# cloudflare/zkp-ecdsa

Hardware: NVIDIA H100
Metric: ZKAttest proofs/sec (higher is better)
Workload: dtype u256/u258 (32-bit limbs, Montgomery)

## Files before the change

__graft_entry__.py:

```python
from __future__ import annotations

import hashlib
import os
import subprocess
import sys

ROOT = os.path.dirname(os.path.abspath(__file__))
CSRC = os.path.join(ROOT, 'zkp_ecdsa_b200', 'csrc')
LIB = os.path.join(ROOT, 'zkp_ecdsa_b200', 'libzkattest.so')
LIB_WAR = os.path.join(ROOT, 'zkp_ecdsa_b200', 'libzkattest_war256.so')
HOSTSIM = os.path.join(ROOT, 'tests', 'hostsim', 'libzkattest_hostsim.so')
HOSTSIM_WAR = os.path.join(ROOT, 'tests', 'hostsim', 'libzkattest_hostsim_war256.so')
PROBE_SRC = os.path.join(ROOT, 'tests', 'probe', 'zk_probe.cu')
PROBE = os.path.join(ROOT, 'tests', 'probe', 'libzkprobe.so')
PROBE_HOST = os.path.join(ROOT, 'tests', 'probe', 'libzkprobe_host.so')
PROBE_JAC_SRC = os.path.join(ROOT, 'tests', 'probe', 'zk_probe_jac.cu')
PROBE_JAC = os.path.join(ROOT, 'tests', 'probe', 'libzkprobe_jac.so')
PROBE_JAC_HOST = os.path.join(ROOT, 'tests', 'probe', 'libzkprobe_jac_host.so')
PROBE_SEED_SRC = os.path.join(ROOT, 'tests', 'probe', 'zk_probe_seed.cu')
PROBE_SEED = os.path.join(ROOT, 'tests', 'probe', 'libzkprobe_seed.so')
PROBE_SEED_HOST = os.path.join(ROOT, 'tests', 'probe', 'libzkprobe_seed_host.so')
PROBE_SHAPE_SRC = os.path.join(ROOT, 'tests', 'probe', 'zk_probe_shape.cu')
PROBE_SHAPE = os.path.join(ROOT, 'tests', 'probe', 'libzkprobe_shape.so')
PROBE_SHAPE_HOST = os.path.join(ROOT, 'tests', 'probe', 'libzkprobe_shape_host.so')
ORACLE_CPU = os.path.join(ROOT, 'oracle', '_ref', 'libzkattest_cpu.so')
ARCH = ['-gencode', 'arch=compute_90a,code=sm_90a']
NVCC_FLAGS = ARCH + ['-O3', '-std=c++17', '-lineinfo',
              '--compiler-options', '-fPIC', '-shared']


def _sources():
    return sorted(os.path.join(CSRC, f) for f in os.listdir(CSRC) if f.endswith(('.cu', '.cuh', '.h', '.inc')))


def _stamp(extra='', files=()):
    h = hashlib.sha256(extra.encode())
    for p in _sources() + [os.path.join(ROOT, 'include', 'zkattest.h')] + list(files):
        h.update(p.encode())
        h.update(open(p, 'rb').read())
    return h.hexdigest()


def _build_if_stale(out, cmd, tag, files=()):
    stamp_file = out + '.stamp'
    stamp = _stamp(' '.join(cmd), files)
    if os.path.exists(out) and os.path.exists(stamp_file) and open(stamp_file).read() == stamp:
        return False
    print(f'[build] {tag}: {" ".join(cmd)}', flush=True)
    tmp = out + '.tmp'
    subprocess.check_call([tmp if c == out else c for c in cmd], cwd=ROOT)
    os.replace(tmp, out)
    open(stamp_file, 'w').write(stamp)
    return True


def build_lib():
    nvcc = os.environ.get('NVCC', '/usr/local/cuda/bin/nvcc')
    cmd = [nvcc] + NVCC_FLAGS + ['-I' + os.path.join(ROOT, 'include'), '-I' + CSRC, '-o', LIB,
                                 os.path.join(CSRC, 'zkattest.cu')]
    return _build_if_stale(LIB, cmd, 'libzkattest.so (sm_90a)')


def build_lib_war():
    nvcc = os.environ.get('NVCC', '/usr/local/cuda/bin/nvcc')
    cmd = [nvcc] + NVCC_FLAGS + ['-DZKA_PG_WAR256', '-I' + os.path.join(ROOT, 'include'), '-I' + CSRC, '-o', LIB_WAR,
                                 os.path.join(CSRC, 'zkattest.cu')]
    return _build_if_stale(LIB_WAR, cmd, 'libzkattest_war256.so (sm_90a)')


def build_hostsim(war=False):
    out = HOSTSIM_WAR if war else HOSTSIM
    os.makedirs(os.path.dirname(out), exist_ok=True)
    cmd = ['g++', '-std=c++17', '-O2', '-DZKA_HOSTSIM'] + (['-DZKA_PG_WAR256'] if war else []) + [
        '-x', 'c++', '-I' + os.path.join(ROOT, 'include'), '-I' + CSRC, '-fPIC', '-shared', '-o', out,
        os.path.join(CSRC, 'zkattest.cu')]
    return _build_if_stale(out, cmd, 'hostsim war256 (tests only)' if war else 'hostsim (tests only)')


def build_probe(host=False, jac=False):
    out = (PROBE_JAC_HOST if host else PROBE_JAC) if jac else (PROBE_HOST if host else PROBE)
    src = PROBE_JAC_SRC if jac else PROBE_SRC
    if host:
        cmd = ['g++', '-std=c++17', '-O2', '-DZKA_HOSTSIM', '-x', 'c++', '-fPIC', '-shared']
    else:
        cmd = [os.environ.get('NVCC', '/usr/local/cuda/bin/nvcc')] + NVCC_FLAGS
    cmd += ['-I' + os.path.join(ROOT, 'include'), '-I' + CSRC, '-o', out, src]
    tag = ('probe_jac' if jac else 'probe') + (' host (tests only)' if host else ' (sm_90a, tests only)')
    return _build_if_stale(out, cmd, tag, [PROBE_SRC, PROBE_JAC_SRC] if jac else [PROBE_SRC])


def build_probe_seed(host=False):
    out = PROBE_SEED_HOST if host else PROBE_SEED
    if host:
        cmd = ['g++', '-std=c++17', '-O2', '-DZKA_HOSTSIM', '-x', 'c++', '-fPIC', '-shared']
    else:
        cmd = [os.environ.get('NVCC', '/usr/local/cuda/bin/nvcc')] + NVCC_FLAGS
    cmd += ['-I' + os.path.join(ROOT, 'include'), '-I' + CSRC, '-o', out, PROBE_SEED_SRC]
    return _build_if_stale(out, cmd, 'probe_seed' + (' host (tests only)' if host else ' (sm_90a, tests only)'), [PROBE_SEED_SRC])


def build_probe_shape(host=False):
    out = PROBE_SHAPE_HOST if host else PROBE_SHAPE
    if host:
        cmd = ['g++', '-std=c++17', '-O2', '-DZKA_HOSTSIM', '-x', 'c++', '-fPIC', '-shared']
    else:
        cmd = [os.environ.get('NVCC', '/usr/local/cuda/bin/nvcc')] + NVCC_FLAGS
    cmd += ['-I' + os.path.join(ROOT, 'include'), '-I' + CSRC, '-o', out, PROBE_SHAPE_SRC]
    return _build_if_stale(out, cmd, 'probe_shape' + (' host (tests only)' if host else ' (sm_90a, tests only)'), [PROBE_SHAPE_SRC])


def build_oracle_cpu():
    src = os.path.join(ROOT, 'oracle', 'cpu', 'zkattest_cpu.cpp')
    hdr = os.path.join(ROOT, 'include', 'zkattest.h')
    if os.path.exists(ORACLE_CPU) and os.path.getmtime(ORACLE_CPU) >= max(os.path.getmtime(src), os.path.getmtime(hdr)):
        return False
    print('[build] oracle/cpu -> oracle/_ref/libzkattest_cpu.so', flush=True)
    subprocess.check_call(['make', '-C', os.path.join(ROOT, 'oracle', 'cpu')])
    return True


def build_tools():
    nvcc = os.environ.get('NVCC', '/usr/local/cuda/bin/nvcc')
    tdir = os.path.join(ROOT, 'tools')
    for name in ('imad_peak', 'mul_peak'):
        src, out = os.path.join(tdir, name + '.cu'), os.path.join(tdir, name)
        if not os.path.exists(src):
            continue
        if os.path.exists(out) and os.path.getmtime(out) >= max(os.path.getmtime(p) for p in _sources() + [src]):
            continue
        cmd = [nvcc] + ARCH + ['-O3', '-std=c++17', '-I' + CSRC,
               '-I' + os.path.join(ROOT, 'include'), '-o', out, src]
        print(f'[build] tools/{name}: {" ".join(cmd)}', flush=True)
        subprocess.check_call(cmd, cwd=ROOT)


def build() -> None:
    from concurrent.futures import ThreadPoolExecutor
    jobs = [build_lib, build_lib_war, build_hostsim, lambda: build_hostsim(war=True), build_oracle_cpu, build_tools,
            build_probe, lambda: build_probe(host=True), lambda: build_probe(jac=True),
            lambda: build_probe(host=True, jac=True), build_probe_seed, lambda: build_probe_seed(host=True),
            build_probe_shape, lambda: build_probe_shape(host=True)]
    with ThreadPoolExecutor(max_workers=min(len(jobs), max(1, (os.cpu_count() or 2)))) as ex:
        for f in [ex.submit(j) for j in jobs]:
            f.result()
    sys.path.insert(0, ROOT)
    import zkp_ecdsa_b200
    import oracle


def smoke() -> None:
    sys.path.insert(0, ROOT)
    import numpy as np
    from zkp_ecdsa_b200 import api, synth
    from oracle import flat
    from oracle import zkattest as OZ
    from oracle.big import Tape

    eng = api.Engine(device=0)
    rnd = synth.params_rnd(1)
    params = eng.generate_params_list(rnd=rnd)
    wl = synth.Workload(B=2, N=8, seed=1)
    tape = synth.random_tape(2, eng.lib.prove_tape_len(8), seed=2)
    res = eng.prove_batch(params, wl.msg_hash, wl.sig, wl.pk, wl.which, wl.ring, tape)
    assert (res.status == 0).all(), res.status
    oparams = OZ.generate_params_list(Tape(rnd))
    for b in range(2):
        pr = OZ.prove_signature_list(oparams, wl.msg_hash[b].tobytes(), wl.sig[b].tobytes(), wl.pk[b].tobytes(),
                                     int(wl.which[b]), wl.ring_ints(), Tape(tape[b].tobytes()))
        assert flat.ser_proof(pr) == res.proof_bytes(b), f'proof {b} differs from the oracle'
    from oracle import seed_tape as ST
    seed = bytes(range(32))
    rs = eng.prove_batch_seeded(params, wl.msg_hash[:1], wl.sig[:1], wl.pk[:1], wl.which[:1], wl.ring,
                                np.frombuffer(seed, np.uint8).reshape(1, 32).copy())
    assert rs.status[0] == 0, rs.status
    pr = OZ.prove_signature_list(oparams, wl.msg_hash[0].tobytes(), wl.sig[0].tobytes(), wl.pk[0].tobytes(),
                                 int(wl.which[0]), wl.ring_ints(), Tape(ST.prove_tape(seed, 80, 3)))
    assert flat.ser_proof(pr) == rs.proof_bytes(0), 'seeded proof differs from the oracle on the expanded tape'
    from zkp_ecdsa_b200 import verify_tape as VT
    vts = eng.lib.verify_tape_len(8, 80)
    ok = np.zeros(2, np.uint8)
    st = np.zeros(2, np.int32)
    eng.lib.verify_batch(params.handle, 2, wl.msg_hash, wl.ring, 8, res.proofs, res.proofs.shape[1], res.proof_len,
                         VT.random_verify_tape(2, vts, 8, 80, seed=3), vts, ok, st)
    assert list(ok) == [1, 1] and not st.any(), (ok, st)
    rw = synth.RingsWorkload(2, [17, 5], [1, 0], seed=5)
    rings = eng.load_rings(rw.rings)
    rt = synth.random_tape(2, eng.lib.prove_tape_len(17), seed=6)
    rr = eng.prove_batch_rings(params, rings, rw.ring_of, rw.msg_hash, rw.sig, rw.pk, rw.which, rt)
    assert (rr.status == 0).all(), rr.status
    for b in range(2):
        pr = OZ.prove_signature_list(oparams, rw.msg_hash[b].tobytes(), rw.sig[b].tobytes(), rw.pk[b].tobytes(),
                                     int(rw.which[b]), rw.ring_ints(int(rw.ring_of[b])), Tape(rt[b].tobytes()))
        assert flat.ser_proof(pr) == rr.proof_bytes(b), f'ring-set proof {b} differs from the oracle'
    rings.close()
    launched = eng.lib.launch_count()
    war = ''
    if os.path.exists(LIB_WAR):
        from oracle.curves import tomEdwards256, war256
        ew = api.Engine(device=0, proof_group='war256')
        pw = ew.generate_params_list(16, rnd=rnd)
        tw = synth.random_tape(1, ew.lib.prove_tape_len(8, 16), seed=4)
        rw = ew.prove_batch(pw, wl.msg_hash[:1], wl.sig[:1], wl.pk[:1], wl.which[:1], wl.ring, tw)
        assert (rw.status == 0).all(), rw.status
        flat.set_proof_group(war256)
        try:
            ow = OZ.generate_params_list(Tape(rnd), 16, war256)
            pr = OZ.prove_signature_list(ow, wl.msg_hash[0].tobytes(), wl.sig[0].tobytes(), wl.pk[0].tobytes(),
                                         int(wl.which[0]), wl.ring_ints(), Tape(tw[0].tobytes()))
            assert flat.ser_proof(pr) == rw.proof_bytes(0), 'war256 proof differs from the oracle'
        finally:
            flat.set_proof_group(tomEdwards256)
        launched += ew.lib.launch_count()
        war = '; war256 build: 1 proof bit-exact'
    print(f'smoke ok: 2 proofs bit-exact vs oracle and accepted by the verifier, 1 seeded proof bit-exact, '
          f'2 ring-set proofs over rings of depths 3 and 5 bit-exact{war}; '
          'kernels launched:', launched)


if __name__ == '__main__':
    build()
    if len(sys.argv) > 1 and sys.argv[1] == 'smoke':
        smoke()
```

zkp_ecdsa_b200/capi.py:

```python
from __future__ import annotations

import ctypes as C
import os
from typing import Optional

import numpy as np

_HERE = os.path.dirname(os.path.abspath(__file__))
DEFAULT_LIB = os.path.join(_HERE, 'libzkattest.so')

SYMBOLS = [
    'zka_init', 'zka_shutdown', 'zka_last_error', 'zka_version', 'zka_launch_count',
    'zka_params_generate', 'zka_params_create', 'zka_params_destroy', 'zka_key_to_int',
    'zka_proof_max_len', 'zka_prove_tape_len', 'zka_verify_tape_len',
    'zka_prove_batch', 'zka_verify_batch',
    'zka_tom_commit_batch', 'zka_p256_mul_batch', 'zka_field_op_batch', 'zka_hash80_batch',
    'zka_get_stream', 'zka_set_profiling', 'zka_profile_reset', 'zka_profile_json', 'zka_config',
    'zka_lanes', 'zka_set_option', 'zka_proofs_pack', 'zka_proofs_unpack', 'zka_verify_batch_ex', 'zka_verify_tape_len_ex',
    'zka_verify_exp_batch', 'zka_verify_membership_batch', 'zka_verify_equality_batch', 'zka_verify_mult_batch',
    'zka_verify_pointadd_batch', 'zka_prove_exp_batch', 'zka_prove_membership_batch',
    'zka_prove_equality_batch', 'zka_prove_mult_batch', 'zka_prove_pointadd_batch', 'zka_stat', 'zka_proof_group', 'zka_set_progress', 'zka_chunk_schedule',
    'zka_prove_batch_seeded', 'zka_verify_batch_seeded', 'zka_seed_tape',
    'zka_rings_create', 'zka_rings_destroy', 'zka_prove_batch_rings', 'zka_prove_batch_rings_seeded', 'zka_verify_batch_rings',
    'zka_verify_batch_rings_seeded', 'zka_prove_batch_hedged', 'zka_prove_batch_rings_hedged', 'zka_hedge_seeds',
# ... 106 lines not shown
            for f in ('zka_verify_equality_batch', 'zka_verify_mult_batch', 'zka_verify_pointadd_batch'):
                getattr(L, f).argtypes = [C.c_void_p, C.c_void_p, C.c_uint32, C.c_void_p, C.c_void_p, C.c_void_p, C.c_size_t,
                                          C.c_void_p, C.c_void_p]
            L.zka_prove_exp_batch.argtypes = [C.c_void_p, C.c_void_p, C.c_uint32] + [C.c_void_p] * 5 + [C.c_size_t, C.c_void_p, C.c_size_t,
                                              C.c_void_p, C.c_void_p]
            L.zka_prove_membership_batch.argtypes = [C.c_void_p, C.c_void_p, C.c_uint32, C.c_void_p, C.c_void_p, C.c_void_p, C.c_uint32,
                                                     C.c_void_p, C.c_size_t, C.c_void_p, C.c_size_t, C.c_void_p, C.c_void_p]
            for f in ('zka_prove_equality_batch', 'zka_prove_mult_batch'):
                getattr(L, f).argtypes = [C.c_void_p, C.c_void_p, C.c_uint32, C.c_void_p, C.c_void_p, C.c_size_t, C.c_void_p, C.c_void_p,
                                          C.c_void_p]
            L.zka_prove_pointadd_batch.argtypes = [C.c_void_p, C.c_void_p, C.c_uint32, C.c_void_p, C.c_void_p, C.c_void_p, C.c_size_t,
                                                   C.c_void_p, C.c_void_p, C.c_void_p]
            L.zka_proofs_pack.argtypes = [C.c_void_p, C.c_uint32, C.c_void_p, C.c_size_t, C.c_void_p, C.c_void_p, C.c_size_t,
                                          C.c_void_p, C.c_void_p]
            L.zka_proofs_unpack.argtypes = [C.c_void_p, C.c_uint32, C.c_void_p, C.c_size_t, C.c_void_p, C.c_void_p, C.c_size_t,
                                            C.c_void_p, C.c_void_p]
        if hasattr(L, 'zka_seed_tape'):
            L.zka_prove_batch_seeded.argtypes = [C.c_void_p, C.c_void_p, C.c_uint32] + [C.c_void_p] * 5 + [C.c_uint32, C.c_void_p,
                                                 C.c_void_p, C.c_size_t, C.c_void_p, C.c_void_p]
            L.zka_verify_batch_seeded.argtypes = [C.c_void_p, C.c_void_p, C.c_uint32, C.c_void_p, C.c_void_p, C.c_uint32, C.c_void_p,
                                                  C.c_size_t, C.c_void_p, C.c_void_p, C.c_uint32, C.c_void_p, C.c_void_p]
            L.zka_seed_tape.argtypes = [C.c_void_p, C.c_int, C.c_uint32, C.c_void_p, C.c_uint32, C.c_uint32, C.c_uint32, C.c_void_p,
                                        C.c_size_t]
        if hasattr(L, 'zka_rings_create'):
            L.zka_rings_create.argtypes = [C.c_void_p, C.c_uint32, C.c_void_p, C.c_void_p, C.POINTER(C.c_void_p)]
            L.zka_rings_destroy.argtypes = [C.c_void_p]
            L.zka_prove_batch_rings.argtypes = [C.c_void_p, C.c_void_p, C.c_void_p, C.c_void_p, C.c_uint32] + [C.c_void_p] * 5 + [
                C.c_size_t, C.c_void_p, C.c_size_t, C.c_void_p, C.c_void_p]
            L.zka_prove_batch_rings_seeded.argtypes = [C.c_void_p, C.c_void_p, C.c_void_p, C.c_void_p, C.c_uint32] + [C.c_void_p] * 6 + [
                C.c_size_t, C.c_void_p, C.c_void_p]
            L.zka_verify_batch_rings.argtypes = [C.c_void_p, C.c_void_p, C.c_void_p, C.c_void_p, C.c_uint32, C.c_void_p, C.c_void_p,
                                                 C.c_size_t, C.c_void_p, C.c_void_p, C.c_size_t, C.c_uint32, C.c_void_p, C.c_void_p]
            L.zka_verify_batch_rings_seeded.argtypes = [C.c_void_p, C.c_void_p, C.c_void_p, C.c_void_p, C.c_uint32, C.c_void_p,
                                                        C.c_void_p, C.c_size_t, C.c_void_p, C.c_void_p, C.c_uint32, C.c_void_p,
                                                        C.c_void_p]
        if hasattr(L, 'zka_hedge_seeds'):
            L.zka_prove_batch_hedged.argtypes = L.zka_prove_batch_seeded.argtypes
            L.zka_prove_batch_rings_hedged.argtypes = L.zka_prove_batch_rings_seeded.argtypes
            L.zka_hedge_seeds.argtypes = [C.c_void_p, C.c_void_p, C.c_uint32] + [C.c_void_p] * 5 + [C.c_uint32, C.c_void_p, C.c_void_p]
            L.zka_hedge_seeds_rings.argtypes = [C.c_void_p, C.c_void_p, C.c_void_p, C.c_void_p, C.c_uint32] + [C.c_void_p] * 6
        ctx = C.c_void_p()
        rc = L.zka_init(device, C.byref(ctx))
        if rc != 0 or not ctx:
            raise ZkaError(f'zka_init(device={device}) failed with {rc}: no usable CUDA device '
                           '(libzkattest has no CPU fallback)')
        self.ctx = ctx
        self.device = device

    def close(self):
        if getattr(self, 'ctx', None):
            self.lib.zka_shutdown(self.ctx)
            self.ctx = None

    def _check(self, rc, what):
        if rc != 0:
            raise ZkaError(f'{what} failed ({rc}): {self.lib.zka_last_error(self.ctx).decode()}')

    def launch_count(self) -> int:
        return int(self.lib.zka_launch_count(self.ctx))

    def stream_ptr(self) -> int:
        return int(self.lib.zka_get_stream(self.ctx) or 0)

    def set_profiling(self, on: bool):
        self._check(self.lib.zka_set_profiling(self.ctx, 1 if on else 0), 'zka_set_profiling')

    def profile_reset(self):
        self._check(self.lib.zka_profile_reset(self.ctx), 'zka_profile_reset')

    def profile(self) -> dict:
        import json
        n = self.lib.zka_profile_json(self.ctx, None, 0)
        buf = C.create_string_buffer(int(n) + 16)
        self.lib.zka_profile_json(self.ctx, buf, len(buf))
        return json.loads(buf.value.decode())

    def config(self) -> dict:
        w, nw, ch = C.c_int(), C.c_int(), C.c_int()
        self._check(self.lib.zka_config(self.ctx, C.byref(w), C.byref(nw), C.byref(ch)), 'zka_config')
        lanes = int(self.lib.zka_lanes(self.ctx)) if hasattr(self.lib, 'zka_lanes') else 1
        cfg = {'tom_w': w.value, 'tom_nwin': nw.value, 'chunk': ch.value, 'lanes': lanes}
        if hasattr(self.lib, 'zka_stat') and self.stat('tom_n_lo') >= 0:
            cfg.update(tom_n_lo=self.stat('tom_n_lo'), tom_fallback=bool(self.stat('tom_fallback')))
        return cfg

    def set_option(self, key: str, value: int):
        self._check(self.lib.zka_set_option(self.ctx, key.encode(), int(value)), f'zka_set_option({key})')

    def chunk_schedule(self, B: int, host_buffers: bool = False):
        off = np.zeros(4096, np.uint32)
        self.lib.zka_chunk_schedule.argtypes = [C.c_void_p, C.c_uint32, C.c_int, C.c_void_p, C.c_uint32]
        n = self.lib.zka_chunk_schedule(self.ctx, B, 1 if host_buffers else 0, _ptr(off), off.size)
        if n < 0:
            raise ZkaError('zka_chunk_schedule')
        return [int(v) for v in off[:n + 1]]

    def set_progress(self, flags: Optional[np.ndarray]):
        self.lib.zka_set_progress.argtypes = [C.c_void_p, C.c_void_p, C.c_uint32]
        if flags is None:
            self._check(self.lib.zka_set_progress(self.ctx, None, 0), 'zka_set_progress')
        else:
            assert flags.dtype == np.uint32 and flags.flags['C_CONTIGUOUS']
            self._check(self.lib.zka_set_progress(self.ctx, _ptr(flags), flags.size), 'zka_set_progress')

    def stat(self, key: str) -> int:
        return int(self.lib.zka_stat(self.ctx, key.encode()))

    def proof_max_len(self, ring_size, sec_level=80): return int(self.lib.zka_proof_max_len(ring_size, sec_level))
    def prove_tape_len(self, ring_size, sec_level=80): return int(self.lib.zka_prove_tape_len(ring_size, sec_level))
    def verify_tape_len(self, ring_size, sec_level=80): return int(self.lib.zka_verify_tape_len(ring_size, sec_level))

    def params_generate(self, rnd: bytes):
        assert len(rnd) == 64
        hn = np.zeros(65, np.uint8)
        hp = np.zeros(self.wp, np.uint8)
        self._check(self.lib.zka_params_generate(self.ctx, _ptr(rnd), _ptr(hn), _ptr(hp)), 'zka_params_generate')
        return hn.tobytes(), hp.tobytes()

    def params_create(self, h_nist: bytes, h_proof: bytes, sec_level: int = 80):
        h = C.c_void_p()
        self._check(self.lib.zka_params_create(self.ctx, _ptr(h_nist), _ptr(h_proof), sec_level, C.byref(h)),
                    'zka_params_create')
        return h

    def params_destroy(self, h):
        self.lib.zka_params_destroy(h)

    def key_to_int(self, pk: np.ndarray):
        count = pk.shape[0]
        out = np.zeros((count, 32), np.uint8)
        st = np.zeros(count, np.int32)
        self._check(self.lib.zka_key_to_int(self.ctx, count, _ptr(pk), _ptr(out), _ptr(st)), 'zka_key_to_int')
        return out, st

    def prove_batch(self, params, B, msg_hash, sig, pk, which, ring, N, tape, tape_stride,
                    proofs, proof_stride, proof_len, status):
        self._check(self.lib.zka_prove_batch(self.ctx, params, B, _ptr(msg_hash), _ptr(sig), _ptr(pk), _ptr(which),
                                             _ptr(ring), N, _ptr(tape), tape_stride, _ptr(proofs), proof_stride,
                                             _ptr(proof_len), _ptr(status)), 'zka_prove_batch')

    def verify_batch(self, params, B, msg_hash, ring, N, proofs, proof_stride, proof_len, tape, tape_stride,
                     ok, status):
        self._check(self.lib.zka_verify_batch(self.ctx, params, B, _ptr(msg_hash), _ptr(ring), N, _ptr(proofs),
                                              proof_stride, _ptr(proof_len), _ptr(tape), tape_stride, _ptr(ok),
                                              _ptr(status)), 'zka_verify_batch')

    def verify_tape_len_ex(self, ring_size, sec_level, samples):
        return int(self.lib.zka_verify_tape_len_ex(ring_size, sec_level, samples))

    def verify_batch_ex(self, params, B, msg_hash, ring, N, proofs, proof_stride, proof_len, tape, tape_stride, ok, status, samples):
        self._check(self.lib.zka_verify_batch_ex(self.ctx, params, B, _ptr(msg_hash), _ptr(ring), N, _ptr(proofs), proof_stride,
                                                 _ptr(proof_len), _ptr(tape), tape_stride, _ptr(ok), _ptr(status), samples),
                    'zka_verify_batch_ex')

    def prove_batch_seeded(self, params, B, msg_hash, sig, pk, which, ring, N, seeds, proofs, proof_stride, proof_len, status):
        self._check(self.lib.zka_prove_batch_seeded(self.ctx, params, B, _ptr(msg_hash), _ptr(sig), _ptr(pk), _ptr(which), _ptr(ring),
                                                    N, _ptr(seeds), _ptr(proofs), proof_stride, _ptr(proof_len), _ptr(status)),
                    'zka_prove_batch_seeded')

    def verify_batch_seeded(self, params, B, msg_hash, ring, N, proofs, proof_stride, proof_len, seeds, samples, ok, status):
        self._check(self.lib.zka_verify_batch_seeded(self.ctx, params, B, _ptr(msg_hash), _ptr(ring), N, _ptr(proofs), proof_stride,
                                                     _ptr(proof_len), _ptr(seeds), samples, _ptr(ok), _ptr(status)),
                    'zka_verify_batch_seeded')

    def seed_tape(self, kind, seeds, ring_size, sec_level=80, samples=20) -> np.ndarray:
        B = seeds.shape[0]
# ... 160 lines not shown
```

zkp_ecdsa_b200/csrc/zk_launch.cuh:

```cuda
#pragma once
#include <stdint.h>
#include <stdlib.h>
#include <string.h>

#include <map>
#include <stdexcept>
#include <string>
#include <typeinfo>
#include <vector>

#include <cxxabi.h>

#if !defined(ZKA_HOSTSIM)
#include <cuda_runtime.h>
#endif

namespace zk {

#if !defined(ZKA_HOSTSIM)

#define ZK_CUDA_CHECK(expr)                                                                   \
  do {                                                                                        \
    cudaError_t _e = (expr);                                                                  \
    if (_e != cudaSuccess)                                                                    \
      throw std::runtime_error(std::string("CUDA error: ") + cudaGetErrorString(_e) + " at " + \
                               __FILE__ + ":" + std::to_string(__LINE__));                    \
  } while (0)

template <class Task>
struct TaskMinBlocks { static constexpr int value = 1; };

template <class Task>
__global__ void __launch_bounds__(128, TaskMinBlocks<Task>::value) zk_task_kernel(int n, Task task) {
  int t = blockIdx.x * blockDim.x + threadIdx.x;
  if (t < n) task(t);
}

struct ProfEntry {
  uint64_t launches = 0;
  double ms = 0.0;
  uint64_t items = 0;
};
struct Stream {
  cudaStream_t s = nullptr;
  uint64_t launches = 0;
  bool profiling = false;
  struct Pending { const char* name; cudaEvent_t e0, e1; long long n; };
  std::vector<Pending> pending;
  std::map<std::string, ProfEntry> prof;
};

inline std::string demangle(const char* n) {
  int status = 0;
  char* d = abi::__cxa_demangle(n, nullptr, nullptr, &status);
  std::string r = (status == 0 && d) ? d : n;
  free(d);
  return r;
}
inline void prof_collect(Stream& st) {
  for (auto& p : st.pending) {
    float ms = 0.f;
    cudaEventElapsedTime(&ms, p.e0, p.e1);
    ProfEntry& e = st.prof[demangle(p.name)];
    e.launches++;
    e.ms += ms;
    e.items += (uint64_t)p.n;
    cudaEventDestroy(p.e0);
    cudaEventDestroy(p.e1);
  }
  st.pending.clear();
}

template <class Task>
inline void launch(Stream& st, long long n, const Task& task) {
  if (n <= 0) return;
  if (n > 0x7fffffffLL) throw std::runtime_error("launch too large");
  const int threads = 128;
  const int blocks = (int)((n + threads - 1) / threads);
  Stream::Pending pd{typeid(Task).name(), nullptr, nullptr, n};
  if (st.profiling) {
    ZK_CUDA_CHECK(cudaEventCreate(&pd.e0));
    ZK_CUDA_CHECK(cudaEventCreate(&pd.e1));
    ZK_CUDA_CHECK(cudaEventRecord(pd.e0, st.s));
  }
  zk_task_kernel<Task><<<blocks, threads, 0, st.s>>>((int)n, task);
  ZK_CUDA_CHECK(cudaGetLastError());
  if (st.profiling) {
    ZK_CUDA_CHECK(cudaEventRecord(pd.e1, st.s));
    st.pending.push_back(pd);
  }
  st.launches++;
}

inline void* dev_alloc(size_t bytes) {
  void* p = nullptr;
  ZK_CUDA_CHECK(cudaMalloc(&p, bytes ? bytes : 1));
  return p;
}
inline void dev_free(void* p) {
  if (p) cudaFree(p);
}
inline void copy_h2d(Stream& st, void* d, const void* h, size_t n) {
  if (n) ZK_CUDA_CHECK(cudaMemcpyAsync(d, h, n, cudaMemcpyDefault, st.s));
}
inline void copy_d2h(Stream& st, void* h, const void* d, size_t n) {
  if (n) ZK_CUDA_CHECK(cudaMemcpyAsync(h, d, n, cudaMemcpyDefault, st.s));
}
inline void copy_d2d(Stream& st, void* d, const void* s, size_t n) {
  if (n) ZK_CUDA_CHECK(cudaMemcpyAsync(d, s, n, cudaMemcpyDeviceToDevice, st.s));
}
inline void copy_d2h_2d(Stream& st, void* h, size_t hpitch, const void* d, size_t dpitch, size_t width, size_t height) {
  if (width && height) ZK_CUDA_CHECK(cudaMemcpy2DAsync(h, hpitch, d, dpitch, width, height, cudaMemcpyDefault, st.s));
}
inline void dev_memset(Stream& st, void* d, int v, size_t n) {
  if (n) ZK_CUDA_CHECK(cudaMemsetAsync(d, v, n, st.s));
}
inline void sync(Stream& st) {
  ZK_CUDA_CHECK(cudaStreamSynchronize(st.s));
  if (!st.pending.empty()) prof_collect(st);
}
struct Event { cudaEvent_t e = nullptr; };
inline void stream_create(Stream& st) {
  if (!st.s) ZK_CUDA_CHECK(cudaStreamCreateWithFlags(&st.s, cudaStreamNonBlocking));
}
inline void stream_destroy(Stream& st) {
  if (st.s) cudaStreamDestroy(st.s);
  st.s = nullptr;
}
inline void ev_record(Event& ev, Stream& st) {
  if (!ev.e) ZK_CUDA_CHECK(cudaEventCreateWithFlags(&ev.e, cudaEventDisableTiming));
  ZK_CUDA_CHECK(cudaEventRecord(ev.e, st.s));
}
inline void ev_wait(Stream& st, Event& ev) {
  if (ev.e) ZK_CUDA_CHECK(cudaStreamWaitEvent(st.s, ev.e, 0));
}
inline void ev_destroy(Event& ev) {
  if (ev.e) cudaEventDestroy(ev.e);
  ev.e = nullptr;
}
inline bool is_device_ptr(const void* p) {
  cudaPointerAttributes a;
  cudaError_t e = cudaPointerGetAttributes(&a, p);
  if (e != cudaSuccess) {
    cudaGetLastError();
    return false;
  }
  return a.type == cudaMemoryTypeDevice || a.type == cudaMemoryTypeManaged;
}

#else

struct ProfEntry {
  uint64_t launches = 0;
  double ms = 0.0;
  uint64_t items = 0;
};
struct Stream {
  uint64_t launches = 0;
  bool profiling = false;
  std::map<std::string, ProfEntry> prof;
};
template <class Task>
inline void launch(Stream& st, long long n, const Task& task) {
  for (long long t = 0; t < n; t++) task((int)t);
  st.launches++;
}
inline void* dev_alloc(size_t bytes) { return calloc(bytes ? bytes : 1, 1); }
inline void dev_free(void* p) { free(p); }
inline void copy_h2d(Stream&, void* d, const void* h, size_t n) { if (n) memcpy(d, h, n); }
inline void copy_d2h(Stream&, void* h, const void* d, size_t n) { if (n) memcpy(h, d, n); }
inline void copy_d2d(Stream&, void* d, const void* s, size_t n) { if (n) memcpy(d, s, n); }
inline void copy_d2h_2d(Stream&, void* h, size_t hpitch, const void* d, size_t dpitch, size_t width, size_t height) {
  for (size_t r = 0; r < height; r++) memcpy((char*)h + r * hpitch, (const char*)d + r * dpitch, width);
}
inline void dev_memset(Stream&, void* d, int v, size_t n) { if (n) memset(d, v, n); }
inline void sync(Stream&) {}
struct Event {};
inline void stream_create(Stream&) {}
inline void stream_destroy(Stream&) {}
inline void ev_record(Event&, Stream&) {}
inline void ev_wait(Stream&, Event&) {}
inline void ev_destroy(Event&) {}
inline bool is_device_ptr(const void*) { return false; }

#endif

struct DevBuf {
  void* p = nullptr;
  size_t cap = 0;
  DevBuf() = default;
  DevBuf(const DevBuf&) = delete;
  DevBuf& operator=(const DevBuf&) = delete;
  ~DevBuf() { dev_free(p); }
  void release() {
    dev_free(p);
    p = nullptr;
    cap = 0;
  }
  template <class T>
  T* get(size_t count) {
    size_t bytes = count * sizeof(T);
    if (bytes > cap) {
      release();
      size_t want = bytes + bytes / 8 + 256;
      p = dev_alloc(want);
      cap = want;
    }
    return reinterpret_cast<T*>(p);
  }
  template <class T>
  T* get_exact(size_t count) {
    release();
    p = dev_alloc(count * sizeof(T));
    cap = count * sizeof(T);
    return reinterpret_cast<T*>(p);
  }
};

struct Cursor {
  DevBuf *next_, *end_;
  template <size_t N>
  explicit Cursor(DevBuf (&pool)[N]) : next_(pool), end_(pool + N) {}
  DevBuf& next() {
    if (next_ == end_) throw std::runtime_error("workspace pool exhausted");
    return *next_++;
  }
  template <class T>
  T* take(size_t count) { return next().get<T>(count); }
  template <class T>
  T* take_if(bool need, size_t count) {
    T* p = take<T>(need ? count : 0);
    return need ? p : nullptr;
  }
};

}
```

zkp_ecdsa_b200/csrc/zk_ops.cuh:

```cuda
#pragma once
#include "zk_curves.cuh"
#include "zk_layout.h"
#include "zk_sha256.cuh"

namespace zk {

#if defined(__CUDA_ARCH__)
#define ZK_SET_STATUS(ptr, code) atomicCAS((int*)(ptr), 0, (int)(code))
#define ZK_POST_MIN(ptr, key) atomicMin((int*)(ptr), (int)(key))
#define ZK_SET_STATUS_OVER(ptr, code, over) \
  do {                                      \
    atomicCAS((int*)(ptr), 0, (int)(code)); \
    atomicCAS((int*)(ptr), (int)(over), (int)(code)); \
  } while (0)
#else
#define ZK_SET_STATUS_OVER(ptr, code, over)              \
  do {                                                   \
    if (*(ptr) == 0 || *(ptr) == (over)) *(ptr) = (code); \
  } while (0)
#define ZK_SET_STATUS(ptr, code) \
  do {                           \
    if (*(ptr) == 0) *(ptr) = (code); \
  } while (0)
#define ZK_POST_MIN(ptr, key)             \
// ... 478 lines not shown
  ZK_HD static void canon2p(uint32_t* r) {
    uint32_t t[9], p2[9];
#pragma unroll
    for (int i = 0; i < 9; i++) p2[i] = (FpTom::p(i) << 1) | (i > 0 ? (FpTom::p(i - 1) >> 31) : 0u);
    uint32_t br = sub_n<9>(t, r, p2);
    csel_n<9>(r, br == 0, t, r);
    br = sub_p<FpTom>(t, r);
    csel_n<9>(r, br == 0, t, r);
  }
  ZK_HD void operator()(int t) const {
    using F = Tomp;
    const int lo = t * chunk;
    int n = count - lo;
    if (n > chunk) n = chunk;
    if (n <= 0) return;
    uint32_t pre[NORM_CHUNK_MAX][9];
    uint32_t acc[9], z[9], h[9], den[9];
    F::set_one(acc);
    for (int k = 0; k < n; k++) {
      const uint32_t* src = proj + (size_t)(lo + k) * stride;
      uint32_t xx[9], yy[9];
      if (e2) {
        tom_ld_efgh(xx, yy, z, h, src);
        F::mul(den, z, h);
      } else {
        tom_ld_xyz(xx, yy, den, src);
      }
      F::mul(acc, acc, den);
      copy_n<9>(pre[k], acc);
    }
    uint32_t inv[9], cxk[9], is2[9], one_plain[9];
    F::inv(inv, acc);
    tom_const(cxk, e2 ? TOM_INVSQRTND : TOM_INVSQRTA);
    tom_const(is2, TOM_INVSQRTND1);
    zero_n<9>(one_plain);
    one_plain[0] = 1;
    for (int k = n - 1; k >= 0; k--) {
      const uint32_t* src = proj + (size_t)(lo + k) * stride;
      uint32_t X[9], Y[9], di[9];
      if (e2) {
        tom_ld_efgh(X, Y, z, h, src);
        F::mul(den, z, h);
        F::mul(X, X, h);
        F::mul(Y, Y, z);
      } else {
        tom_ld_xyz(X, Y, den, src);
      }
      if (k > 0) F::mul(di, inv, pre[k - 1]); else copy_n<9>(di, inv);
      F::mul(inv, inv, den);
      if (bytes) {
        uint32_t Dp[9], cx[9], cy[9];
        F::mul(Dp, di, one_plain);
        F::mul(cx, X, cxk);
        F::mul(cx, cx, Dp);
        F::mul(cy, Y, Dp);
        canon2p(cx);
        canon2p(cy);
        store_point_words<9, 33>(bytes + (size_t)(lo + k) * BSTRIDE, 0x04u, cx, cy);
      }
      if (aff && ((lo + k) % aff_mod) < aff_lim) {
        uint32_t x[9], y[9];
        F::mul(x, X, di);
        if (e2) F::mul(x, x, is2);
        F::mul(y, Y, di);
        uint32_t* a = aff + (size_t)(lo + k) * TOM_AFF_WORDS;
        st<9>(a, x);
        st<9>(a + 9, y);
      }
    }
  }
};

ZK_HD void tom2_ld_entry(TomPre& q, const uint32_t* tab, const FbShape& sh, int j, uint32_t d, bool neg) {
  tom_ld_pre(q, tab + (sh.offset(j) + d) * TOM_PRE_WORDS);
  tom2_pre_neg(q, neg);
}

struct TomCommitTask {
  const uint32_t* jv;
  const uint32_t* jr;
  const uint32_t* gtab;
  const uint32_t* htab;
  uint32_t* proj;
  FbShape sh;
  int xyz = 0;
  ZK_HD void operator()(int t) const {
    uint32_t v[8], r[8];
    ld<8>(v, jv + (size_t)t * 8);
    ld<8>(r, jr + (size_t)t * 8);
    uint32_t cv = 0, cr = 0;
    bool nv, nr;
    TomPre q;
    uint32_t dv = signed_digit(v, 0, sh, cv, nv);
    tom2_ld_entry(q, gtab, sh, 0, dv, nv);
    TomPt acc;
    tom2_from_pre(acc, q);
    for (int j = 0;; j++) {
      const uint32_t dr = signed_digit(r, j, sh, cr, nr);
      tom2_ld_entry(q, htab, sh, j, dr, nr);
      if (j == sh.nwin - 1) break;
      tom2_madd<true>(acc, acc, q);
      dv = signed_digit(v, j + 1, sh, cv, nv);
      tom2_ld_entry(q, gtab, sh, j + 1, dv, nv);
      tom2_madd<true>(acc, acc, q);
    }
    if (xyz) {
      tom2_madd<false>(acc, acc, q);
      tom_st_xyz(proj + (size_t)t * TOM_PROJ_WORDS, acc.x, acc.y, acc.z);
    } else {
      TomEfgh e;
      tom2_madd_end(e, acc, q);
      tom_st_efgh(proj + (size_t)t * TOM_E2_WORDS, e);
    }
  }
};

struct TomCommitGTask {
  const uint32_t* jv;
  const uint32_t* gtab;
  uint32_t* ext;
  FbShape sh;
  GpartLayout lay;
  ZK_HD void operator()(int t) const {
    const int row = t / lay.gparts(), jb = lay.job_of_gpart(row, t % lay.gparts());
    if (jb < 0) return;
    uint32_t v[8];
    ld<8>(v, jv + ((size_t)row * lay.jobs() + jb) * 8);
    uint32_t carry = 0;
    bool neg;
    TomPre q;
    const uint32_t d0 = signed_digit(v, 0, sh, carry, neg);
    tom2_ld_entry(q, gtab, sh, 0, d0, neg);
    TomPt acc;
    tom2_from_pre<TompCommit>(acc, q);
#pragma unroll 1
    for (int j = 1; j < sh.nwin; j++) {
      const uint32_t d = signed_digit(v, j, sh, carry, neg);
      tom2_ld_entry(q, gtab, sh, j, d, neg);
      tom2_madd<true, TompCommit>(acc, acc, q);
    }
    uint32_t* o = ext + (size_t)t * TOM_EXT_WORDS;
    st<9>(o, acc.x); st<9>(o + 9, acc.y); st<9>(o + 18, acc.t); st<9>(o + 27, acc.z);
  }
};
struct TomCommitHTask {
  const uint32_t* jv;
  const uint32_t* jr;
  const uint32_t* gtab;
  const uint32_t* htab;
  const uint32_t* ext;
  uint32_t* proj;
  FbShape sh;
  GpartLayout lay;
  ZK_HD void operator()(int t) const {
    const int row = t / lay.jobs(), g = lay.gpart_of_job(row, t % lay.jobs());
    uint32_t v[8], r[8];
    ld<8>(v, jv + (size_t)t * 8);
    TomPt acc;
    TomPre q;
    if (g < 0 || scalar_le_one(v)) {
      tom2_ld_entry(q, gtab, sh, 0, v[0], false);
      tom2_from_pre<TompCommit>(acc, q);
    } else {
      const uint32_t* s = ext + ((size_t)row * lay.gparts() + g) * TOM_EXT_WORDS;
      ld<9>(acc.x, s); ld<9>(acc.y, s + 9); ld<9>(acc.t, s + 18); ld<9>(acc.z, s + 27);
    }
    ld<8>(r, jr + (size_t)t * 8);
    uint32_t carry = 0;
    bool neg;
#pragma unroll 1
    for (int j = 0; j < sh.nwin - 1; j++) {
      const uint32_t d = signed_digit(r, j, sh, carry, neg);
      tom2_ld_entry(q, htab, sh, j, d, neg);
      tom2_madd<true, TompCommit>(acc, acc, q);
    }
    const uint32_t d = signed_digit(r, sh.nwin - 1, sh, carry, neg);
    tom2_ld_entry(q, htab, sh, sh.nwin - 1, d, neg);
    TomEfgh e;
    tom2_madd_end<TompCommit>(e, acc, q);
    tom_st_efgh(proj + (size_t)t * TOM_E2_WORDS, e);
  }
};

#if !defined(ZKA_HOSTSIM) && defined(ZKA_COMMIT_MINBLOCKS)
template <> struct TaskMinBlocks<TomCommitHTask> { static constexpr int value = ZKA_COMMIT_MINBLOCKS; };
template <> struct TaskMinBlocks<TomCommitGTask> { static constexpr int value = ZKA_COMMIT_MINBLOCKS; };
template <> struct TaskMinBlocks<TomCommitTask> { static constexpr int value = ZKA_COMMIT_MINBLOCKS; };
#endif

#endif

enum : int { GK_BLOCK_BITS = 10 };
ZK_HD int gk_block_bits(int n) { return n < GK_BLOCK_BITS ? n : GK_BLOCK_BITS; }
ZK_HD void gk_block_sum(uint32_t* acc, const uint32_t* ring_m, const uint32_t (*fz)[8], const uint32_t (*fo)[8], int n,
                        int k, uint32_t blk, const uint32_t* vw) {
  using F = Tomq;
  uint32_t P[21][8];
  F::set_one(P[n]);
  for (int j = n - 1; j >= k; j--) F::mul(P[j], P[j + 1], ((blk >> (j - k)) & 1u) ? fo[j] : fz[j]);
  for (int j = k - 1; j >= 0; j--) F::mul(P[j], P[j + 1], fz[j]);
  zero_n<8>(acc);
  const size_t base = (size_t)blk << k;
  const uint32_t cnt = 1u << k;
  for (uint32_t l = 0;;) {
    uint32_t vi[8], term[8];
    ld<8>(vi, ring_m + (base + l) * 8);
    if (vw) F::sub(vi, vw, vi);
    F::mul(term, vi, P[0]);
    F::add(acc, acc, term);
    l++;
    if (l == cnt) break;
    int tz = 0;
    while (!((l >> tz) & 1u)) tz++;
    F::mul(P[tz], P[tz + 1], fo[tz]);
    for (int j = tz - 1; j >= 0; j--) F::mul(P[j], P[j + 1], fz[j]);
  }
}

ZK_HD bool hash_pt_fetch(uint32_t* t, const uint8_t* p, int len) {
  if (((size_t)p & 3) || len < 64 || len > 68) return false;
  if (aligned16(p)) {
#pragma unroll
    for (int j = 0; j < 4; j++) ld4(t + 4 * j, p + 16 * j);
    t[16] = len > 64 ? *reinterpret_cast<const uint32_t*>(p + 64) : 0u;
    return true;
  }
  const uint32_t* q = reinterpret_cast<const uint32_t*>(p);
#pragma unroll
  for (int j = 0; j < 17; j++) t[j] = (4 * j < len) ? q[j] : 0u;
  return true;
}
template <class Src>
ZK_HD void hash_points80(uint32_t* c3, const Src& src, int npts) {
  Sha256 h;
  h.init();
  uint32_t nx[17], cu[17];
  int nlen = 0;
  const uint8_t* np = npts > 0 ? src(0, nlen) : nullptr;
  bool nfast = npts > 0 && hash_pt_fetch(nx, np, nlen);
  for (int i = 0; i < npts; i++) {
    const uint8_t* p = np;
    const int len = nlen;
    const bool fast = nfast;
#pragma unroll
    for (int j = 0; j < 17; j++) cu[j] = nx[j];
    if (i + 1 < npts) {
      np = src(i + 1, nlen);
      nfast = hash_pt_fetch(nx, np, nlen);
    }
    if (fast) h.feed17(cu, len);
    else h.update(p, len);
  }
  h.final80(c3);
}

ZK_HD void challenge_to_limbs(uint32_t* r, const uint32_t* c3) {
  zero_n<8>(r);
  r[0] = c3[0]; r[1] = c3[1]; r[2] = c3[2];
}

// ... 125 lines not shown
```

zkp_ecdsa_b200/csrc/zk_ops_war.cuh:

```cuda
#pragma once

#define WEI_PT WarPt
#define WEI_AFF WarAff
#define WEI_JAC WarJac
#define WEI_F Warp
#define WEI_FN(n) war_##n
#define WEI_T(n) War##n
#include "zk_weier_ops.inc"
#undef WEI_PT
#undef WEI_AFF
#undef WEI_JAC
#undef WEI_F
#undef WEI_FN
#undef WEI_T

struct TomNormTask {
  const uint32_t* proj;
  uint32_t* aff;
  uint8_t* bytes;
  int count;
  int chunk;
  int e2;
  int aff_mod, aff_lim;
  int stride;
  ZK_HD void operator()(int t) const {
    using F = Warp;
    const int lo = t * chunk;
    int n = count - lo;
    if (n > chunk) n = chunk;
    if (n <= 0) return;
    uint32_t pre[NORM_CHUNK_MAX][8];
    uint32_t acc[8], z[8], one[8];
    F::set_one(one);
    copy_n<8>(acc, one);
    for (int k = 0; k < n; k++) {
      ld<8>(z, proj + (size_t)(lo + k) * stride + 16);
      if (is_zero_n<8>(z)) copy_n<8>(z, one);
      F::mul(acc, acc, z);
      copy_n<8>(pre[k], acc);
    }
    uint32_t inv[8];
    F::inv(inv, acc);
    for (int k = n - 1; k >= 0; k--) {
      const uint32_t* src = proj + (size_t)(lo + k) * stride;
      ld<8>(z, src + 16);
      const bool isinf = is_zero_n<8>(z);
      if (isinf) copy_n<8>(z, one);
      uint32_t zi[8];
      if (k > 0) F::mul(zi, inv, pre[k - 1]); else copy_n<8>(zi, inv);
      F::mul(inv, inv, z);
      uint32_t X[8], Y[8], x[8], y[8];
      ld<8>(X, src);
      ld<8>(Y, src + 8);
      F::mul(x, X, zi);
      F::mul(y, Y, zi);
      if (aff && ((lo + k) % aff_mod) < aff_lim) {
        uint32_t* a = aff + (size_t)(lo + k) * TOM_AFF_WORDS;
        st<8>(a, x);
        st<8>(a + 8, y);
      }
      if (bytes) {
        uint32_t cx[8], cy[8];
        F::from_mont(cx, x);
        F::from_mont(cy, y);
        if (isinf) { zero_n<8>(cx); zero_n<8>(cy); }
        store_point_words<8, 32>(bytes + (size_t)(lo + k) * BSTRIDE, isinf ? 0x00u : 0x04u, cx, cy);
      }
    }
  }
};

struct TomCommitTask {
  const uint32_t* jv;
  const uint32_t* jr;
  const uint32_t* gtab;
  const uint32_t* htab;
  uint32_t* proj;
  FbShape sh;
  int xyz = 0;
  ZK_HD void operator()(int t) const {
    uint32_t v[8], r[8];
    ld<8>(v, jv + (size_t)t * 8);
    ld<8>(r, jr + (size_t)t * 8);
    WarJac aj;
    war_set_identity_jac(aj);
    war_accum_fixed_jac(aj, gtab, v, sh.w);
    war_accum_fixed_jac(aj, htab, r, sh.w);
    WarPt acc;
    war_jac_to_hom(acc, aj);
    war_st_proj(proj + (size_t)t * TOM_PROJ_WORDS, acc);
  }
};
ZK_HD void war_gpart(WarPt& acc, const uint32_t* gtab, const uint32_t* v, int w) {
  WarJac aj;
  war_set_identity_jac(aj);
  war_accum_fixed_jac(aj, gtab, v, w);
  war_jac_to_hom(acc, aj);
}
struct TomCommitGTask {
  const uint32_t* jv;
  const uint32_t* gtab;
  uint32_t* ext;
  FbShape sh;
  GpartLayout lay;
  ZK_HD void operator()(int t) const {
    const int row = t / lay.gparts(), jb = lay.job_of_gpart(row, t % lay.gparts());
    if (jb < 0) return;
    uint32_t v[8];
    ld<8>(v, jv + ((size_t)row * lay.jobs() + jb) * 8);
    WarPt acc;
    war_gpart(acc, gtab, v, sh.w);
    war_st_proj(ext + (size_t)t * TOM_EXT_WORDS, acc);
  }
};
struct TomCommitHTask {
  const uint32_t* jv;
  const uint32_t* jr;
  const uint32_t* gtab;
  const uint32_t* htab;
  const uint32_t* ext;
  uint32_t* proj;
  FbShape sh;
  GpartLayout lay;
  ZK_HD void operator()(int t) const {
    const int row = t / lay.jobs(), g = lay.gpart_of_job(row, t % lay.jobs());
    uint32_t v[8], r[8];
    ld<8>(v, jv + (size_t)t * 8);
    ld<8>(r, jr + (size_t)t * 8);
    WarPt acc;
    if (g < 0 || scalar_le_one(v)) war_gpart(acc, gtab, v, sh.w);
    else war_ld_proj(acc, ext + ((size_t)row * lay.gparts() + g) * TOM_EXT_WORDS);
    war_accum_fixed(acc, htab, r, sh.w);
    war_st_proj(proj + (size_t)t * TOM_PROJ_WORDS, acc);
  }
};
```

zkp_ecdsa_b200/csrc/zk_prove.cuh:

```cuda
#pragma once
#include "zk_sigma.cuh"

namespace zk {

struct ProveCtx {
  int B;
  int S;
  int N;
  int n;
  int M;
  FbShape tom;
  int mode;
  int head_len;
  const uint8_t* base;
  const uint8_t* s_in;
  const uint8_t* q_in;
  uint32_t* base_aff;
  const uint8_t* msg_hash;
  const uint8_t* sig;
  const uint8_t* pk;
  const uint32_t* which;
  uint32_t* which_s;
  const uint8_t* tape;
  size_t tape_stride;
  uint32_t tape_draws;
  const uint32_t* ring_m;
  const uint32_t* ring_of;
  const uint32_t* ring_base;
  const uint32_t* ring_size;
  const uint32_t* ring_depth;
  const uint32_t* g_tab8;
  const uint32_t* h_tab8;
  int h_w;
  const uint32_t* g_tabw;
  int g_w;
  const uint32_t* tg_tab;
  const uint32_t* th_tab;
  const uint8_t* tg_bytes;
  uint32_t* s1;
  uint32_t* pk_aff;
  uint32_t* q_aff;
  uint8_t* q_inf;
  uint32_t* r_aff;
  uint8_t* r_bytes;
  uint32_t* u12;
  uint32_t* tab_of;
  uint32_t* tab_rep;
  uint32_t* tab_count;
  uint32_t* rpows;
  uint32_t* rrows;
  uint32_t* rtab;
  uint32_t* pa_T;
  uint32_t* pa_A;
  uint32_t* pa_T_aff;
  uint8_t* pa_T_inf;
  uint32_t* pa_A_aff;
  uint8_t* pa_A_bytes;
  uint8_t* pa_A_inf;
  uint32_t *s1_jv, *s1_jr, *s1_proj, *s1_aff;
  uint8_t* s1_bytes;
  uint32_t* chal;
  uint32_t* zcount;
  uint32_t* item_base;
  uint32_t* item_total;
  uint32_t* rep_off;
  uint32_t* gk_off;
  uint32_t* item_b;
  uint32_t* item_i;
  uint32_t* item_k;
  uint32_t* pb_T1;
  uint32_t* pb_T1_aff;
  uint8_t* pb_T1_inf;
  uint32_t *s2_jv, *s2_jr, *s2_proj, *s2_aff;
  uint8_t* s2_bytes;
  uint32_t* item_inv;
  uint32_t* secrets;
  uint32_t* item_chal;
  uint32_t* gk_dv;
  uint32_t* gk_part;
  uint32_t* gk_lag;
  uint32_t* gk_x;
  uint8_t* proofs;
  size_t proof_stride;
  uint32_t* proof_len;
  int32_t* status;

  ZK_HD size_t s2_job(size_t item, int j) const { return item * JOBS_PER_ITEM + j; }
  ZK_HD size_t s2_der(size_t item, int j) const { return (size_t)M * JOBS_PER_ITEM + item * DERS_PER_ITEM + j; }
  ZK_HD size_t s2_gk(size_t b, int j) const { return (size_t)M * (JOBS_PER_ITEM + DERS_PER_ITEM) + b * 4 * n + j; }
  ZK_HD size_t s2_count() const { return (size_t)M * (JOBS_PER_ITEM + DERS_PER_ITEM) + (size_t)B * 4 * n; }
  ZK_HD size_t s1_pt(size_t b, int j) const { return b * (2 + 2 * S) + j; }
  ZK_HD const uint8_t* tape_of(int b) const { return tape + (size_t)b * tape_stride; }
  ZK_HD const uint32_t* ring_of_row(int b) const { return ring_of ? ring_m + (size_t)8 * ring_base[ring_of[b]] : ring_m; }
  ZK_HD uint32_t ring_size_row(int b) const { return ring_of ? ring_size[ring_of[b]] : (uint32_t)N; }
// ... 1114 lines not shown
```

zkp_ecdsa_b200/csrc/zk_verify.cuh:

```cuda
#pragma once
#include "zk_prove.cuh"

namespace zk {

enum : int {
  V_SAMPLES = 20,
  V_ENT_PER_SAMPLE = 2 + PA_ENTRIES,
  V_SEG = 20,
  V_ENT_SEG = V_SEG * V_ENT_PER_SAMPLE + 2,
  V_IDX_PAD = 96,
  V_PART_WORDS = 7 * 8,
  MSM_C = 6,
  MSM_NWIN = 43,
  MSM_C_N = 4,
  MSM_NWIN_N = 65,
  AGG_SKIP = 0,
  AGG_TOM_PASS = 1,
  AGG_NIST_PASS = 2,
  AGG_CTL_WORDS = 4,
  AGG_W_GK = 0, AGG_W_W = 1, AGG_W_N = 2, AGG_WT = 3,
};

enum : int { VK_NONE = 0x7fffffff, VK_PARAMS = 0, VK_FIRST_DRAW = 1, VK_T_INF = 2, VK_DRAWS = 3 };
ZK_HD int vkey(int sample, int phase, int code) { return ((sample + 1) << 8) | (phase << 4) | code; }

ZK_LAYOUT_FN size_t verify_tape_len(int n, int , int K = V_SAMPLES) {
  return (size_t)32 * (2 * n + 1) + V_IDX_PAD + (size_t)32 * 25 * K;
}

struct VerifyCtx {
  int B, S, N, n;
  int K;
  int mode;
  const uint8_t* q_ext;
  FbShape tom;
  const uint8_t* msg_hash;
  const uint8_t* proofs;
  size_t proof_stride;
  const uint32_t* proof_len;
  const uint8_t* tape;
  size_t tape_stride;
  const uint32_t* ring_m;
  const uint32_t* ring_of;
  const uint32_t* ring_base;
  const uint32_t* ring_depth;
  const uint32_t* g_tab8;
  const uint32_t* h_tab8;
  int h_w;
  const uint32_t* tg_tab;
  const uint32_t* th_tab;
  const uint8_t* tg_bytes;
  uint32_t* rep_off;
  uint32_t* gk_off;
  uint32_t* tagbits;
  uint32_t* chal;
  uint32_t* chal_full;
  uint8_t* gk_ok_len;
  uint8_t* gk_tape_bad;
  uint32_t* r_aff;
  uint32_t* q_aff;
  uint8_t* q_inf;
  uint32_t* rpows;
  uint32_t* rrows;
  uint32_t* rtab;
  uint32_t* samp_idx;
  uint32_t* samp_draw;
  uint32_t* sp_T;
  uint32_t* sp_T_aff;
  uint8_t* sp_T_inf;
  uint32_t *ta_jv, *ta_jr, *ta_proj, *ta_aff;
  uint32_t *td_proj, *td_aff;
  uint8_t* td_bytes;
  uint32_t* item_chal;
  uint32_t* ent_scalar;
  uint32_t* ent_off;
  uint32_t* ent_pre;
  uint32_t* ent_cnt;
  uint32_t* part;
  uint32_t* nent_scalar;
  uint32_t* nent_aff;
  uint8_t* nent_skip;
  uint32_t* gk_scalar;
  uint32_t* gk_part;
  uint32_t* gk_pre;
  uint32_t *fx_jv, *fx_jr, *fx_proj;
  uint32_t* nfix;
  uint32_t* nfix_k;
  uint32_t* win_w;
  uint32_t* win_g;
  uint32_t* win_n;
  uint8_t* id_flags;
  int32_t* vkey;
  const uint32_t* agg_ctl;
  uint8_t* ok;
  int32_t* status;

  ZK_HD int ent_tom() const { return K * V_ENT_PER_SAMPLE + 2; }
  ZK_HD int ent_nist() const { return K + 1; }
  ZK_HD int segs() const { return (K + V_SEG - 1) / V_SEG; }
  ZK_HD const uint8_t* proof_of(int b) const { return proofs + (size_t)b * proof_stride; }
  ZK_HD const uint8_t* tape_of(int b) const { return tape + (size_t)b * tape_stride; }
  ZK_HD const uint32_t* ring_of_row(int b) const { return ring_of ? ring_m + (size_t)8 * ring_base[ring_of[b]] : ring_m; }
  ZK_HD int n_row(int b) const { return ring_of ? (int)ring_depth[ring_of[b]] : n; }
  ZK_HD size_t gk_tape_bytes(int b) const { return mode == 1 ? 0 : (size_t)32 * (2 * n_row(b) + 1); }
  ZK_HD const uint8_t* exp_tape(int b) const { return tape_of(b) + gk_tape_bytes(b) + V_IDX_PAD; }
  ZK_HD size_t ta_pt(size_t sample, int j) const { return sample * 2 + j; }
  ZK_HD size_t td_pt(size_t sample, int j) const { return sample * DERS_PER_ITEM + j; }
};

struct VLayoutTask {
  VerifyCtx c;
  ZK_HD void operator()(int b) const {
    using Fn = P256n;
    using Fp = P256p;
    c.status[b] = ZKA_OK;
    c.vkey[b] = VK_NONE;
    c.ok[b] = 0;
    const uint8_t* pr = c.proof_of(b);
// ... 1000 lines not shown
```

zkp_ecdsa_b200/csrc/zkattest.cu:

```cuda
#include "zkattest.h"

#include <math.h>
#include <stdio.h>

#include <algorithm>
#include <atomic>
#include <cmath>
#include <mutex>
#include <chrono>
#include <memory>
#include <thread>
#include <string>
#include <vector>

#include "zk_check.cuh"
#include "zk_launch.cuh"
#include "zk_prove.cuh"
#include "zk_seed.cuh"
#include "zk_verify_agg.cuh"

namespace zk {
struct ParsePointsTask {
  const uint8_t* nist;
  const uint8_t* tom;
// ... 194 lines not shown
    const int b = t / pieces, j = t % pieces;
    const size_t o = (size_t)16 * j;
    if (o >= len[b]) return;
    const size_t po = (size_t)off[b] + o;
    if (po + 16 > cap) return;
    uint8_t* r = rows + (size_t)b * stride + o;
    uint8_t* q = packed + po;
    if (dir == 0) { for (int i = 0; i < 16; i++) q[i] = o + i < stride ? r[i] : 0; }
    else { for (int i = 0; i < 16; i++) if (o + i < stride) r[i] = q[i]; }
  }
};
struct PackCopy16Task {
  uint8_t* rows;
  size_t stride;
  const uint32_t* len;
  const uint64_t* off;
  uint8_t* packed;
  size_t cap;
  int pieces;
  int dir;
  ZK_HD void operator()(int t) const {
    const int b = t / pieces, j = t % pieces;
    const size_t o = (size_t)16 * j;
    if (o >= len[b]) return;
    const size_t po = (size_t)off[b] + o;
    if (po + 16 > cap) return;
    U4* r = reinterpret_cast<U4*>(rows + (size_t)b * stride + o);
    U4* q = reinterpret_cast<U4*>(packed + po);
    if (dir == 0) *q = *r; else *r = *q;
  }
};

}

using namespace zk;

namespace {

struct FixedTable {
  DevBuf buf;
  uint32_t* tab = nullptr;
};

}

struct Lane {
  Stream st;
  Stream cs_in, cs_out;
  Event ev_small[2], ev_tape[2], ev_done[2], ev_out[2];
  Stream aux[2];
  Event ev_fork, ev_join[2];
  DevBuf w[52];
  DevBuf in[2][10], out[2][3];
  DevBuf agg[9], agg_tom[5 + 2 * AGG_MAX_LEVELS], agg_nist[5 + 2 * AGG_MAX_LEVELS];
  DevBuf chk[5], chk_count;
  std::string err;
  ~Lane() {
    for (int i = 0; i < 2; i++) {
      ev_destroy(ev_small[i]); ev_destroy(ev_tape[i]); ev_destroy(ev_done[i]); ev_destroy(ev_out[i]);
    }
    ev_destroy(ev_fork); ev_destroy(ev_join[0]); ev_destroy(ev_join[1]);
    stream_destroy(cs_in);
    stream_destroy(cs_out);
    stream_destroy(aux[0]);
    stream_destroy(aux[1]);
    stream_destroy(st);
  }
};

struct zka_ctx : Lane {
  int device = 0;
  std::vector<std::unique_ptr<Lane>> extra;
  int nlanes = 3;
  DevBuf ring_in, ring_m;
  DevBuf ring_leaves, ring_digest;
  Lane& lane(int i) { return i == 0 ? *this : *extra[i - 1]; }
#if defined(ZKA_PG_WAR256)
  FbShape tom = fb_uniform(22);
#else
  FbShape tom = fb_lookups(11);
#endif
  size_t tom_table_max = 0;
  bool tom_fallback = false;
  int chunk = 4096;
  int host_chunk = 2048;
  volatile uint32_t* progress = nullptr;
  uint32_t progress_cap = 0;
  int agg = 1;
  int agg_c = 0;
  uint64_t agg_pass = 0, agg_fail = 0;
  int self_check = 0;
  uint64_t self_check_rows = 0, self_check_fail = 0;
  std::mutex stat_mu;
  std::mutex copy_mu;
  int agg_c_last = 0;
  bool tape_split = true;
  int p256_hw = 20;
  FixedTable g8;
  FixedTable gw;
  FixedTable tg;
  DevBuf tg_bytes;
  DevBuf lag;
  int lag_n = -1;
};

struct zka_params {
  zka_ctx* ctx = nullptr;
  uint32_t sec_level = 80;
  FixedTable h8;
  int h_w = 20;
  FixedTable th;
  uint8_t h_nist[65];
  uint8_t h_proof[WP];
  uint8_t hedge_digest[32];
};

struct zka_rings {
  zka_ctx* ctx = nullptr;
  uint32_t R = 0;
  std::vector<uint32_t> size;
  std::vector<int> depth;
  DevBuf ring_m, ring_base, ring_size, ring_depth;
  DevBuf lag;
  DevBuf ring_digest;
};

namespace {

int fail(zka_ctx* ctx, int code, const std::string& msg) {
  if (ctx) ctx->err = msg;
  return code;
}
template <class Fn>
int guarded(zka_ctx* ctx, Fn&& body) {
  try {
    return body();
  } catch (const std::exception& e) {
    return fail(ctx, ZKA_E_CUDA, e.what());
  }
}

template <class Src>
void agg_msm(Stream& st, Cursor A, const Src& src, const AggPlan& pl, const uint32_t* ctl, const uint32_t** rootA,
             const uint32_t** rootB) {
  const AggDigits& D = pl.D;
  const int nwin = D.nwin, nb = D.nb, nseg = (nb + 1 + AGG_SEG - 1) / AGG_SEG;
  const size_t cap = (size_t)src.slots();
  uint32_t* hist = A.take<uint32_t>((size_t)nwin * (nb + 1));
  uint32_t* bstart = A.take<uint32_t>((size_t)nwin * (nb + 2));
  uint32_t* segtot = A.take<uint32_t>((size_t)nwin * nseg);
  uint32_t* sorted = A.take<uint32_t>((size_t)nwin * cap);
  uint32_t* bsum = A.take<uint32_t>((size_t)nwin * nb * Src::PTW);
  dev_memset(st, hist, 0, (size_t)nwin * (nb + 1) * 4);
  launch(st, (long long)cap, AggHistTask<Src>{src, D, ctl, hist});
  launch(st, (long long)nwin * nseg, AggSegSumTask{ctl, hist, segtot, nb, nseg});
  launch(st, nwin, AggSegScanTask{ctl, segtot, nseg});
  launch(st, (long long)nwin * nseg, AggOffsetsTask{ctl, segtot, hist, bstart, nb, nseg});
  launch(st, (long long)cap, AggScatterTask<Src>{src, D, ctl, hist, sorted, cap});
  launch(st, (long long)nwin * nb, AggBucketTask<Src>{src, ctl, bstart, sorted, bsum, cap, nb});
  const uint32_t *inA = bsum, *inB = nullptr;
  int nin = nb, ll = 0;
  for (int lv = 0; lv < pl.levels; lv++) {
    const int nout = nin >> pl.lm[lv];
    uint32_t* oA = A.take<uint32_t>((size_t)nwin * nout * Src::PTW);
    uint32_t* oB = A.take<uint32_t>((size_t)nwin * nout * Src::PTW);
    launch(st, (long long)nwin * nout, AggLevelTask<Src>{ctl, inA, inB, oA, oB, nin, pl.lm[lv], ll, nwin, D.top_shift});
    inA = oA; inB = oB; nin = nout; ll += pl.lm[lv];
  }
  *rootA = inA;
  *rootB = inB;
}

int ceil_log2(uint32_t v) {
  int n = 0;
  while ((1ull << n) < v) n++;
  return n;
}


static int g_norm_slots = 132 * 4;
static bool g_norm_model = true;
inline int norm_chunk_for(long long count, int per_point = 11) {
  if (!g_norm_model) {
    long long c = count / 100000;
    if (c < 8) c = 8;
    if (c > NORM_CHUNK_MAX) c = NORM_CHUNK_MAX;
    return (int)c;
  }
  int best = 8;
  long long best_cost = -1;
  for (int c = 8; c <= NORM_CHUNK_MAX; c++) {
    const long long threads = (count + c - 1) / c, ctas = (threads + 127) / 128;
    const long long waves = (ctas + g_norm_slots - 1) / g_norm_slots;
    const long long cost = waves * ((long long)per_point * c + 70);
    if (best_cost < 0 || cost < best_cost) { best_cost = cost; best = c; }
  }
  return best;
}
inline void launch_p256_norm(Stream& st, const uint32_t* proj, uint32_t* aff, uint8_t* bytes, uint8_t* inf, long long count) {
  if (count <= 0) return;
  const int ch = norm_chunk_for(count, bytes ? 7 : 5);
  launch(st, (count + ch - 1) / ch, P256NormTask{proj, aff, bytes, inf, (int)count, ch});
}
inline void launch_tom_norm(Stream& st, const uint32_t* proj, uint32_t* aff, uint8_t* bytes, long long count, int e2,
                            int aff_mod = 1, int aff_lim = 1, int stride = 0) {
  if (count <= 0) return;
  const int ch = norm_chunk_for(count);
  if (stride == 0) stride = e2 ? TOM_E2_WORDS : TOM_PROJ_WORDS;
  launch(st, (count + ch - 1) / ch, TomNormTask{proj, aff, bytes, (int)count, ch, e2, aff_mod, aff_lim, stride});
}

void build_p256_tab(zka_ctx* ctx, const uint32_t* base_aff_dev, FixedTable& out, int w) {
  Stream& st = ctx->st;
  const int nwin = fb_windows(w);
  const size_t E = (size_t)fb_entries(w), count = (size_t)nwin * E;
  DevBuf pows, rows;
  uint32_t* d_pows = pows.get<uint32_t>((size_t)nwin * P256_PROJ_WORDS);
  uint32_t* d_rows = rows.get<uint32_t>(count * P256_PROJ_WORDS);
  out.tab = out.buf.get<uint32_t>(count * P256_AFF_WORDS);
  launch(st, 1, P256PowsTask{base_aff_dev, nullptr, d_pows, 1, nwin, w});
  if (w > 9) {
    DevBuf hi;
    const int nh = 1 << (w - 9);
    uint32_t* d_hi = hi.get<uint32_t>((size_t)nwin * nh * P256_PROJ_WORDS);
    launch(st, nwin, P256RowsHiTask{d_pows, d_hi, d_rows, w});
    launch(st, (long long)nwin * nh, P256RowsLoTask{d_pows, d_hi, d_rows, w});
    sync(st);
  } else {
    launch(st, nwin, P256RowsTask{d_pows, d_rows, w});
  }
  launch_p256_norm(st, d_rows, out.tab, nullptr, nullptr, (long long)(count));
  sync(st);
}
uint32_t* alloc_tom_tab(zka_ctx* ctx, DevBuf& buf) {
  const size_t words = ctx->tom.total() * TOM_PRE_WORDS;
  if (ctx->tom_table_max && words * sizeof(uint32_t) > ctx->tom_table_max)
    throw std::runtime_error("proof-group fixed-base table of " + std::to_string(words * sizeof(uint32_t)) + " bytes exceeds ZKA_TOM_TABLE_MAX");
  return buf.get_exact<uint32_t>(words);
}
#if defined(ZKA_PG_WAR256)
void build_tom_tab(zka_ctx* ctx, const uint32_t* base_aff_dev, FixedTable& out) {
  Stream& st = ctx->st;
  const int w = ctx->tom.w, nwin = ctx->tom.nwin;
  const size_t E = (size_t)fb_entries(w), count = (size_t)nwin * E;
  DevBuf pows, rows;
  uint32_t* d_pows = pows.get<uint32_t>((size_t)nwin * P256_PROJ_WORDS);
  uint32_t* d_rows = rows.get<uint32_t>(count * P256_PROJ_WORDS);
  out.tab = alloc_tom_tab(ctx, out.buf);
  launch(st, 1, WarPowsTask{base_aff_dev, nullptr, d_pows, 1, nwin, w});
  if (w > 9) {
    DevBuf hi;
    const int nh = 1 << (w - 9);
    uint32_t* d_hi = hi.get<uint32_t>((size_t)nwin * nh * P256_PROJ_WORDS);
    launch(st, nwin, WarRowsHiTask{d_pows, d_hi, d_rows, w});
    launch(st, (long long)nwin * nh, WarRowsLoTask{d_pows, d_hi, d_rows, w});
    sync(st);
  } else {
    launch(st, nwin, WarRowsTask{d_pows, d_rows, w});
  }
  {
    const int ch = norm_chunk_for((long long)count, 5);
    launch(st, ((long long)count + ch - 1) / ch, WarNormTask{d_rows, out.tab, nullptr, nullptr, (int)count, ch});
  }
  sync(st);
}
#else
void build_tom_tab(zka_ctx* ctx, const uint32_t* base_aff_dev, FixedTable& out) {
  Stream& st = ctx->st;
  const FbShape sh = ctx->tom;
  out.tab = alloc_tom_tab(ctx, out.buf);
  DevBuf pows, rows, hi;
  uint32_t* d_pows = pows.get<uint32_t>((size_t)sh.nwin * 36);
  uint32_t* d_rows = rows.get<uint32_t>(sh.entries(sh.nwin - 1) * TOM_PROJ_WORDS);
  launch(st, 1, TomPowsTask{base_aff_dev, d_pows, 1, sh});
  const bool two_level = sh.w > 9;
  uint32_t* d_hi = nullptr;
  if (two_level) {
    d_hi = hi.get<uint32_t>(tom_hi_offset(sh, sh.nwin) * 36);
    launch(st, sh.nwin, TomRowsHiTask{d_pows, d_hi, sh});
  }
  for (int j = 0; j < sh.nwin; j++) {
    const size_t ne = sh.entries(j);
    const uint32_t* pw = d_pows + (size_t)j * 36;
    if (two_level) {
      const int nh = 1 << (sh.width(j) - 9);
      launch(st, nh + 1, TomRowsLoTask{pw, d_hi + tom_hi_offset(sh, j) * 36, d_rows, nh});
    } else {
      launch(st, 1, TomRowsTask{pw, d_rows, sh.width(j)});
    }
    launch(st, (long long)(ne + 15) / 16, TomTabE2Task{d_rows, out.tab + sh.offset(j) * TOM_PRE_WORDS, (int)ne});
  }
  sync(st);
}

#endif

template <class T>
const T* stage_in(Stream& st, DevBuf& buf, const T* p, size_t count) {
  if (!p || count == 0) return p;
  if (is_device_ptr(p)) return p;
  T* d = buf.get<T>(count);
  copy_h2d(st, d, p, count * sizeof(T));
  return d;
}

template <class T>
struct Output {
  T* dst;
  size_t width;
  bool dev;
  Output(T* p, size_t width) : dst(p), width(width), dev(is_device_ptr(p)) {}
  T* rows(DevBuf& stage, uint32_t b0, size_t rows) const { return dev ? dst + b0 * width : stage.get<T>(rows * width); }
  void copy_back(Stream& st, uint32_t b0, const T* d, size_t rows) const {
    if (!dev) copy_d2h(st, dst + b0 * width, d, rows * width * sizeof(T));
  }
  void copy_back_2d(Stream& st, uint32_t b0, const T* d, size_t rows, size_t bytes) const {
    if (!dev) copy_d2h_2d(st, dst + b0 * width, width * sizeof(T), d, width * sizeof(T), bytes, rows);
  }
};

std::vector<uint32_t> chunk_schedule(uint32_t B, uint32_t cmax, int lanes, bool taper) {
  std::vector<uint32_t> off{0};
  auto r32 = [](uint32_t v) { return v < 32 ? std::max<uint32_t>(v, 1) : ((v + 31) & ~31u); };
  if (lanes > 1) {
    uint32_t per = r32((B + (uint32_t)lanes - 1) / (uint32_t)lanes);
    cmax = std::min(cmax, std::max<uint32_t>(per, 256));
  }
  uint32_t done = 0;
  auto push = [&](uint32_t n) { n = std::min(n, B - done); if (n) { done += n; off.push_back(done); } };
  if (taper && cmax >= 1024 && B >= 3 * cmax) {
    const uint32_t q = r32(cmax / 4), h = r32(cmax / 2);
    push(q);
    push(h);
    const uint32_t mid = B - done - (h + q);
    const uint32_t nm = (mid + cmax - 1) / cmax;
    const uint32_t each = r32((mid + nm - 1) / nm);
    for (uint32_t i = 0; i + 1 < nm; i++) push(each);
    push(B - done - (h + q));
    push(h);
    push(q);
  } else {
    const uint32_t nk = (B + cmax - 1) / cmax;
    const uint32_t each = r32((B + nk - 1) / nk);
    while (done < B) push(each);
  }
  return off;
}

#if !defined(ZKA_HOSTSIM)
void CUDART_CB progress_cb(void* p) { *reinterpret_cast<volatile uint32_t*>(p) = 1u; }
void notify_progress(Stream& st, volatile uint32_t* flag) { ZK_CUDA_CHECK(cudaLaunchHostFunc(st.s, progress_cb, (void*)flag)); }
#else
void notify_progress(Stream&, volatile uint32_t* flag) { *flag = 1u; }
// ... 59 lines not shown
    skip(v.proofs, proof_stride); skip(v.proof_len, 1); skip(v.status, 1);
    return v;
  }
};
struct VerifyRows {
  const uint8_t *msg_hash{}, *proofs{}, *tape{}, *seeds{}, *q_ext{};
  const uint32_t *proof_len{}, *ring_of{};
  size_t proof_stride{}, tape_stride{};
  uint8_t* ok{}; int32_t* status{};
  VerifyRows() = default;
  VerifyRows(const uint8_t* proofs, size_t stride, const uint32_t* len, uint8_t* ok, int32_t* status)
      : proofs(proofs), proof_len(len), proof_stride(stride), ok(ok), status(status) {}
  VerifyRows at(size_t r0) const {
    VerifyRows v = *this;
    auto skip = [r0](auto*& p, size_t width) { if (p) p += r0 * width; };
    skip(v.msg_hash, 32); skip(v.proofs, proof_stride); skip(v.proof_len, 1); skip(v.tape, tape_stride); skip(v.seeds, 32);
    skip(v.ring_of, 1); skip(v.q_ext, NP); skip(v.ok, 1); skip(v.status, 1);
    return v;
  }
};

struct RingSrc {
  const uint8_t* ring; uint32_t N;
  const zka_rings* set; int n;
  static RingSrc one(const uint8_t* ring, uint32_t N) { return {ring, N, nullptr, ceil_log2(N)}; }
  static RingSrc pass(const zka_rings* set, int n) { return {nullptr, 0, set, n}; }
  static RingSrc none(int n) { return {nullptr, 2, nullptr, n}; }
  const uint32_t* prepare(zka_ctx* ctx, bool lagrange, bool digest = false) const {
    if (!set && !ring) return nullptr;
    if (set) return (const uint32_t*)set->ring_m.p;
    const uint32_t* ring_m = prep_ring(ctx, ctx->st, ring, N, n, lagrange, digest);
    sync(ctx->st);
    return ring_m;
  }
  const uint8_t* digests(const zka_ctx* ctx) const { return (const uint8_t*)(set ? set->ring_digest.p : ctx->ring_digest.p); }
  template <class Ctx>
  void fill(Ctx& c, const uint32_t* ring_m, const uint32_t* ring_of) const {
    c.ring_m = ring_m;
    if (!set) return;
    c.ring_of = ring_of;
    c.ring_base = (const uint32_t*)set->ring_base.p;
    c.ring_depth = (const uint32_t*)set->ring_depth.p;
    if constexpr (std::is_same<Ctx, ProveCtx>::value) {
      c.ring_size = (const uint32_t*)set->ring_size.p;
      c.gk_lag = (uint32_t*)set->lag.p;
    }
  }
};

template <class Check, class Pass>
int ring_passes(zka_ctx* ctx, const RingSrc& ring, const uint32_t* ring_of, uint32_t B, Check check, Pass pass) {
  if (ring.set && ring.set->ctx != ctx) return fail(ctx, ZKA_E_ARG, "ring set of another context");
  if (B == 0) return 0;
  return guarded(ctx, [&] {
    if (!ring.set) {
      if (ring.N < 2 || ring.N > (1u << 20)) return fail(ctx, ZKA_E_ARG, "ring size must be in [2, 2^20]");
      const int rc = check(ring.n);
      return rc ? rc : pass(ring);
    }
    std::vector<uint32_t> h(B);
    if (is_device_ptr(ring_of)) {
      copy_d2h(ctx->st, h.data(), ring_of, (size_t)B * 4);
      sync(ctx->st);
    } else {
      memcpy(h.data(), ring_of, (size_t)B * 4);
    }
    const std::vector<int>& depth = ring.set->depth;
    int nmax = 0;
    for (uint32_t b = 0; b < B; b++) {
      if (h[b] >= ring.set->R) return fail(ctx, ZKA_E_ARG, "ring_of[i] >= number of rings in the set");
      nmax = std::max(nmax, depth[h[b]]);
    }
    const int rc = check(nmax);
    return rc ? rc : pass(RingSrc::pass(ring.set, nmax));
  });
}

int gk_blocks(int n) { return 1 << (n - gk_block_bits(n)); }

ProveCtx prove_ctx(const zka_ctx* ctx, const zka_params* P, int B, int S, int N, int n) {
  ProveCtx c;
  memset(&c, 0, sizeof(c));
  c.B = B; c.S = S; c.N = N; c.n = n;
  c.tom = ctx->tom;
  c.g_tab8 = ctx->g8.tab; c.h_tab8 = P->h8.tab; c.h_w = P->h_w;
  c.g_tabw = ctx->gw.tab; c.g_w = ctx->p256_hw;
  c.tg_tab = ctx->tg.tab; c.th_tab = P->th.tab;
  c.tg_bytes = (const uint8_t*)ctx->tg_bytes.p;
  c.gk_lag = (uint32_t*)ctx->lag.p;
  return c;
}
VerifyCtx verify_ctx(const zka_ctx* ctx, const zka_params* P, int B, int S, int N, int n, int K, int mode) {
  VerifyCtx c;
  memset(&c, 0, sizeof(c));
  c.B = B; c.S = S; c.N = N; c.n = n; c.K = K; c.mode = mode;
  c.tom = ctx->tom;
  c.g_tab8 = ctx->g8.tab; c.h_tab8 = P->h8.tab; c.h_w = P->h_w;
  c.tg_tab = ctx->tg.tab; c.th_tab = P->th.tab;
  c.tg_bytes = (const uint8_t*)ctx->tg_bytes.p;
  return c;
}

void prove_store1(Stream& st, const ProveCtx& c) {
  const long long n1 = (long long)c.B * (2 + 2 * c.S);
  launch(st, n1, JobsATask{c});
  launch(st, n1, TomCommitTask{c.s1_jv, c.s1_jr, c.tg_tab, c.th_tab, c.s1_proj, c.tom});
  launch_tom_norm(st, c.s1_proj, c.s1_aff, c.s1_bytes, n1, 1);
}
size_t prove_gext_words(const ProveCtx& c) { return ((size_t)c.M * GJOBS_PER_ITEM + (size_t)c.B * 2 * c.n) * TOM_EXT_WORDS; }
void prove_items_gk(Stream& st, const ProveCtx& c, uint32_t* gext, bool items, bool gk) {
  const long long M = c.M, nj = M * JOBS_PER_ITEM, nd = M * DERS_PER_ITEM;
  const long long Bn = (long long)c.B * c.n, ng = 4 * Bn;
  const int nblk = gk_blocks(c.n);
  const size_t g0 = c.s2_gk(0, 0);
  const GpartLayout item_lay{0, nullptr, nullptr}, gk_lay{c.n, c.ring_of, c.ring_depth};
  uint32_t* gk_ext = gext + (size_t)M * GJOBS_PER_ITEM * TOM_EXT_WORDS;
  if (items) {
    launch(st, (M + ITEM_INV_CHUNK - 1) / ITEM_INV_CHUNK, ItemInvTask{c});
    launch(st, M, ItemScalarsTask{c});
  }
  if (gk) {
    launch(st, Bn, GkJobsTask{c});
    launch(st, Bn * nblk, GkPolyTask{c});
    if (nblk > 1) launch(st, Bn, GkPolyReduceTask{c});
    launch(st, Bn, GkCdJobsTask{c});
  }
  if (items) {
    launch(st, M * GJOBS_PER_ITEM, TomCommitGTask{c.s2_jv, c.tg_tab, gext, c.tom, item_lay});
    launch(st, nj, TomCommitHTask{c.s2_jv, c.s2_jr, c.tg_tab, c.th_tab, gext, c.s2_proj, c.tom, item_lay});
  }
  if (gk) {
    launch(st, 2 * Bn, TomCommitGTask{c.s2_jv + g0 * 8, c.tg_tab, gk_ext, c.tom, gk_lay});
    launch(st, ng, TomCommitHTask{c.s2_jv + g0 * 8, c.s2_jr + g0 * 8, c.tg_tab, c.th_tab, gk_ext, c.s2_proj + g0 * TOM_E2_WORDS,
                                  c.tom, gk_lay});
  }
  if (items) {
    launch_tom_norm(st, c.s2_proj, c.s2_aff, c.s2_bytes, nj, 1, JOBS_PER_ITEM, 2);
    launch(st, M, DerivedTask{c});
    launch_tom_norm(st, c.s2_proj + nj * TOM_E2_WORDS, nullptr, c.s2_bytes + nj * BSTRIDE, nd, 0, 1, 1, TOM_E2_WORDS);
  }
  if (gk) launch_tom_norm(st, c.s2_proj + g0 * TOM_E2_WORDS, nullptr, c.s2_bytes + g0 * BSTRIDE, ng, 1);
  if (items) {
    launch(st, M * HASHES_PER_ITEM, ItemHashTask{c});
    launch(st, M * 7, ItemEmitTask{c});
  }
}
void verify_gk(Stream& st, const VerifyCtx& c, uint32_t* gk_offs) {
  const int nblk = gk_blocks(c.n), ngk = 4 * c.n + 1;
  if (nblk > 1) launch(st, (long long)c.B * nblk, VGkSumTask{c});
  launch(st, c.B, VGkTask{c});
  launch(st, (long long)c.B * ngk, VGkOffsetsTask{c, gk_offs});
}

const uint32_t* verify_chunk(zka_ctx* ctx, Lane& ln, VerifyCtx& c, uint32_t b0, bool agg, int* agg_c) {
  Stream& st = ln.st;
  const int Bc = c.B, S = c.S, K = c.K, n = c.n, mode = c.mode;
  const size_t ns = (size_t)Bc * K;
  const int ET = c.ent_tom(), EN = c.ent_nist(), SG = c.segs();
  const int ngk = 4 * n + 1;
  Cursor w(ln.w);
  c.rep_off = w.take<uint32_t>((size_t)Bc * S);
  c.gk_off = w.take<uint32_t>(Bc);
  c.tagbits = w.take<uint32_t>((size_t)Bc * 3);
  c.chal = w.take<uint32_t>((size_t)Bc * 3);
  c.gk_ok_len = w.take<uint8_t>(Bc);
  c.r_aff = w.take<uint32_t>((size_t)Bc * 16);
  c.q_aff = w.take<uint32_t>((size_t)Bc * 16);
  c.q_inf = w.take<uint8_t>(Bc);
  c.rpows = w.take<uint32_t>((size_t)Bc * RT_NWIN * P256_PROJ_WORDS);
  c.rrows = w.take<uint32_t>((size_t)Bc * RT_ENTRIES * P256_PROJ_WORDS);
  c.rtab = w.take<uint32_t>((size_t)Bc * RT_ENTRIES * P256_AFF_WORDS);
  c.samp_idx = w.take<uint32_t>(ns);
  c.samp_draw = w.take<uint32_t>(ns);
  c.sp_T = w.take<uint32_t>(ns * P256_PROJ_WORDS);
  c.sp_T_aff = w.take<uint32_t>(ns * 16);
  c.sp_T_inf = w.take<uint8_t>(ns);
  c.ta_jv = w.take<uint32_t>(ns * 2 * 8);
  c.ta_jr = w.take<uint32_t>(ns * 2 * 8);
  c.ta_proj = w.take<uint32_t>(ns * 2 * TOM_E2_WORDS);
  c.ta_aff = w.take<uint32_t>(ns * 2 * TOM_AFF_WORDS);
  c.td_proj = w.take<uint32_t>(ns * DERS_PER_ITEM * TOM_PROJ_WORDS);
  c.td_aff = w.take<uint32_t>(ns * DERS_PER_ITEM * TOM_AFF_WORDS);
  c.td_bytes = w.take<uint8_t>(ns * DERS_PER_ITEM * BSTRIDE);
  c.item_chal = w.take<uint32_t>(ns * HASHES_PER_ITEM * 3);
  c.ent_scalar = w.take<uint32_t>((size_t)Bc * ET * 8);
  c.ent_off = w.take<uint32_t>((size_t)Bc * ET);
  c.ent_pre = w.take<uint32_t>((size_t)Bc * ET * TOM_PRE_WORDS);
  c.ent_cnt = w.take<uint32_t>(ns);
  c.part = w.take<uint32_t>(ns * V_PART_WORDS);
  c.fx_jv = w.take<uint32_t>((size_t)Bc * 2 * 8);
  c.fx_jr = w.take<uint32_t>((size_t)Bc * 2 * 8);
  c.fx_proj = w.take<uint32_t>((size_t)Bc * 2 * TOM_PROJ_WORDS);
  c.nfix = w.take<uint32_t>((size_t)Bc * P256_PROJ_WORDS);
  c.id_flags = w.take<uint8_t>((size_t)Bc * 3);
  c.gk_tape_bad = w.take_if<uint8_t>(mode == 0, Bc);
  c.vkey = w.take<int32_t>(Bc);
  c.nent_scalar = w.take<uint32_t>((size_t)Bc * EN * 8);
  c.nent_aff = w.take<uint32_t>((size_t)Bc * EN * 16);
  c.nent_skip = w.take<uint8_t>((size_t)Bc * EN);
  c.gk_scalar = w.take<uint32_t>((size_t)Bc * ngk * 8);
  c.gk_pre = w.take<uint32_t>((size_t)Bc * ngk * TOM_PRE_WORDS);
  uint32_t* gk_offs = w.take<uint32_t>((size_t)Bc * ngk);
  c.win_w = w.take<uint32_t>((size_t)Bc * SG * MSM_NWIN * 36);
  c.win_g = w.take<uint32_t>((size_t)Bc * MSM_NWIN * 36);
  c.win_n = w.take<uint32_t>((size_t)Bc * MSM_NWIN_N * P256_PROJ_WORDS);
  c.gk_part = w.take_if<uint32_t>(gk_blocks(n) > 1, (size_t)Bc * gk_blocks(n) * 8);
  const size_t agg_tape_len = verify_tape_len(n, S, K);
  const int agg_tp = agg_tape_pieces(agg_tape_len), agg_np = agg_tp + K + 1;
  uint32_t* agg_wt = w.take_if<uint32_t>(agg, (size_t)Bc * AGG_WT * 8);
  uint32_t* agg_dig = w.take_if<uint32_t>(agg, (size_t)Bc * agg_np * 8);
  c.chal_full = w.take_if<uint32_t>(agg, (size_t)Bc * 8);
  c.nfix_k = w.take_if<uint32_t>(agg, (size_t)Bc * 16);

  launch(st, Bc, VLayoutTask{c});
  launch(st, (long long)Bc * (S + 1), VValidateTask{c});
  {
    const bool fork = !st.profiling;
    Stream& sr = fork ? ln.aux[0] : st;
    if (fork) { ev_record(ln.ev_fork, st); ev_wait(sr, ln.ev_fork); }
    launch(sr, Bc, P256PowsTask{c.r_aff, nullptr, c.rpows, Bc, RT_NWIN, RT_W});
    launch(sr, (long long)Bc * RT_NWIN, P256RowsSignedTask{c.rpows, c.rrows});
    launch_p256_norm(sr, c.rrows, c.rtab, nullptr, nullptr, (long long)Bc * RT_ENTRIES);
    launch(st, Bc, VChallengeTask{c});
    if (fork) { ev_record(ln.ev_join[0], sr); ev_wait(st, ln.ev_join[0]); }
  }
  const bool gk_fork = mode == 0 && !st.profiling;
  if (gk_fork) {
    ev_record(ln.ev_fork, st);
    ev_wait(ln.aux[1], ln.ev_fork);
  }
  if (agg) {
    Stream& sw = gk_fork ? ln.aux[1] : st;
    launch(sw, (long long)Bc * agg_np, AggPieceTask{c, agg_tape_len, agg_tp, agg_np, agg_dig});
    launch(sw, Bc, AggWeightTask{c, c.chal_full, agg_dig, b0, agg_np, agg_wt});
  }
  if (gk_fork) {
    verify_gk(ln.aux[1], c, gk_offs);
    ev_record(ln.ev_join[1], ln.aux[1]);
  }
  launch(st, (long long)ns, VSampleP256Task{c});
  launch_p256_norm(st, c.sp_T, c.sp_T_aff, nullptr, c.sp_T_inf, (long long)(ns));
  launch(st, (long long)ns, VSampleJobsTask{c});
  launch(st, (long long)ns * 2, TomCommitTask{c.ta_jv, c.ta_jr, c.tg_tab, c.th_tab, c.ta_proj, c.tom});
  launch_tom_norm(st, c.ta_proj, c.ta_aff, nullptr, (long long)(ns * 2), 1);
  launch(st, (long long)ns, VDerivedTask{c});
  launch_tom_norm(st, c.td_proj, nullptr, c.td_bytes, (long long)(ns * DERS_PER_ITEM), 0);
  launch(st, (long long)ns * HASHES_PER_ITEM, VItemHashTask{c});
  dev_memset(st, c.ent_off, 0, (size_t)Bc * ET * 4);
  launch(st, (long long)ns, VRelationsTask{c});
  if (mode == 0) {
    if (gk_fork) ev_wait(st, ln.ev_join[1]);
    else verify_gk(st, c, gk_offs);
  }
  launch(st, Bc, VReduceTask{c});
  launch(st, (long long)Bc * ET, VParseEntriesTask{c.proofs, c.proof_stride, c.ent_off, c.ent_pre, ET});
  if (mode == 0) launch(st, (long long)Bc * ngk, VParseEntriesTask{c.proofs, c.proof_stride, gk_offs, c.gk_pre, ngk});
  launch(st, (long long)Bc * 2, TomCommitTask{c.fx_jv, c.fx_jr, c.tg_tab, c.th_tab, c.fx_proj, c.tom, 1});
  uint32_t* ctl = nullptr;
  if (agg) {
    Cursor A(ln.agg);
    const int fgroups = (Bc * 2 + 63) / 64, ngroups = (Bc + 31) / 32, ngroups2 = (ngroups + 31) / 32;
    ctl = A.take<uint32_t>(AGG_CTL_WORDS);
#if !defined(ZKA_PG_WAR256)
    uint32_t* tpart = A.take<uint32_t>((size_t)Bc * (K + 2) * 2 * PG_EXT_WORDS);
#endif
    uint32_t* fpart = A.take<uint32_t>((size_t)fgroups * 16);
    uint32_t* fjv = A.take<uint32_t>(8);
    uint32_t* fjr = A.take<uint32_t>(8);
    uint32_t* fproj = A.take<uint32_t>(TOM_PROJ_WORDS);
    uint32_t* nfix_w = A.take<uint32_t>((size_t)Bc * P256_PROJ_WORDS);
    uint32_t* npart = A.take<uint32_t>((size_t)ngroups * P256_PROJ_WORDS);
    uint32_t* npart2 = A.take_if<uint32_t>(ngroups > 32, (size_t)ngroups2 * P256_PROJ_WORDS);
    dev_memset(st, ctl, 0, AGG_CTL_WORDS * 4);
    launch(st, Bc, AggGateTask{c, ctl});
    const AggTomSrc tsrc{c.ent_scalar, c.ent_pre, c.ent_cnt, c.gk_scalar, c.gk_pre, Bc, ET, K, ngk, agg_wt};
    const AggNistSrc nsrc{c.nent_scalar, c.nent_aff, c.nent_skip, Bc, EN, agg_wt};
    const bool fork = !st.profiling;
    Stream& sa = fork ? ln.aux[0] : st;
    Stream& sb = fork ? ln.aux[1] : st;
    if (fork) {
      ev_record(ln.ev_fork, st);
      ev_wait(sa, ln.ev_fork);
      ev_wait(sb, ln.ev_fork);
    }
#if !defined(ZKA_PG_WAR256)
    launch(sa, (long long)Bc * (K + 2) * 2, AggTorsionPartTask{tsrc, ctl, tpart});
    launch(sa, (long long)Bc * 2, AggTorsionTask{tpart, ctl, K});
#endif
    const AggPlan tp = agg_plan((double)Bc * (0.5 * K * V_ENT_PER_SAMPLE + 2 + ngk), ctx->agg_c);
    const AggPlan np = agg_plan((double)Bc * EN, 0);
    if (agg_c) *agg_c = tp.D.c;
    const uint32_t *tA, *tB, *nA, *nB;
    agg_msm(st, Cursor(ln.agg_tom), tsrc, tp, ctl, &tA, &tB);
    agg_msm(sb, Cursor(ln.agg_nist), nsrc, np, ctl, &nA, &nB);
    launch(st, fgroups, AggFixPartTask{ctl, c.fx_jv, c.fx_jr, agg_wt, fpart, Bc});
    launch(st, 1, AggFixSumTask{ctl, fpart, fjv, fjr, fgroups});
    launch(st, 1, TomCommitTask{fjv, fjr, c.tg_tab, c.th_tab, fproj, c.tom, 1});
    launch(sb, Bc, AggNistFixWeightTask{ctl, c.nfix_k, agg_wt, c.rtab, c.h_tab8, c.h_w, nfix_w});
    launch(sb, ngroups, AggNistFixPartTask{ctl, nfix_w, npart, Bc});
    int nleft = ngroups;
    const uint32_t* nsum = npart;
    if (nleft > 32) {
      launch(sb, ngroups2, AggNistFixPartTask{ctl, npart, npart2, nleft});
      nsum = npart2;
      nleft = ngroups2;
    }
    if (fork) {
      ev_record(ln.ev_join[0], sa);
      ev_record(ln.ev_join[1], sb);
      ev_wait(st, ln.ev_join[0]);
      ev_wait(st, ln.ev_join[1]);
    }
    launch(st, 33, AggFinalTask{ctl, tA, tB, fproj, tp.D.nwin, tp.D.c, nA, nB, nsum, np.D.nwin, np.D.c, nleft});
    c.agg_ctl = ctl;
  }
  {
    const int nW = Bc * SG * MSM_NWIN, nWp = (nW + 31) & ~31, nG = Bc * MSM_NWIN;
    launch(st, (long long)nWp + nG,
           MsmTomWindowBothTask{MsmTomWindowTask{c.ent_scalar, c.ent_pre, c.ent_cnt, ET, K, V_ENT_PER_SAMPLE, 2, V_SEG, SG, c.win_w},
                                MsmTomWindowTask{c.gk_scalar, c.gk_pre, nullptr, ngk, 0, 0, mode == 0 ? ngk : 0, V_SEG, 1, c.win_g}, nW, nWp, nG, ctl});
  }
  launch(st, (long long)Bc * MSM_NWIN_N, MsmP256WindowTask{c.nent_scalar, c.nent_aff, c.nent_skip, c.win_n, EN, ctl});
  {
    const int Bp = (Bc + 31) & ~31;
    launch(st, 3ll * Bp, MsmCombineAllTask{MsmTomCombineTask{c.win_g, c.fx_proj, c.id_flags, 2, 0, 0},
                                           MsmTomCombineTask{c.win_w, c.fx_proj, c.id_flags, 2, 1, 1, SG},
                                           MsmP256CombineTask{c.win_n, c.nfix, c.id_flags}, Bc, Bp, ctl});
  }
  launch(st, Bc, VFinalTask{c});
  return ctl;
}

void check_chunk(zka_ctx* ctx, const zka_params* P, Lane& ln, const ProveCtx& pc, const ProveRows& in, const RingSrc& ring,
                 const uint32_t* ring_m, const uint8_t* key, size_t key_stride, int key_len, uint32_t b0, uint32_t* counts) {
  Stream& st = ln.st;
  const int Bc = pc.B, S = pc.S, n = pc.n;
  const size_t tape_stride = verify_tape_len(n, S, S);
  Cursor k(ln.chk);
  uint8_t* seeds = k.take<uint8_t>((size_t)Bc * 32);
  uint8_t* todo = k.take<uint8_t>(Bc);
  uint8_t* tape = k.take<uint8_t>((size_t)Bc * tape_stride);
  uint8_t* ok = k.take<uint8_t>(Bc);
  int32_t* vstatus = k.take<int32_t>(Bc);
  launch(st, Bc, CheckSeedTask{key, key_stride, key_len, pc.status, seeds, todo});
  VerifyCtx c = verify_ctx(ctx, P, Bc, S, pc.N, n, S, 0);
  c.msg_hash = in.msg_hash;
  c.proofs = pc.proofs;
  c.proof_stride = pc.proof_stride;
  c.proof_len = pc.proof_len;
  c.tape = tape;
  c.tape_stride = tape_stride;
  ring.fill(c, ring_m, in.ring_of);
  const SeedVerifyTapeTask vt{seeds, tape, tape_stride, n, S, S, c.ring_of, c.ring_depth};
  launch(st, (long long)Bc * vt.slots(), vt);
  c.ok = ok;
  c.status = vstatus;
  verify_chunk(ctx, ln, c, b0, ctx->agg != 0, nullptr);
  launch(st, (long long)Bc * FIN_PARTS, CheckReleaseTask{todo, ok, vstatus, pc.proofs, pc.proof_stride, pc.proof_len, pc.status, counts});
}

}

extern "C" {

int zka_version(void) { return 1; }

const char* zka_last_error(const zka_ctx* ctx) { return ctx ? ctx->err.c_str() : "null context"; }

uint64_t zka_launch_count(const zka_ctx* ctx) {
  if (!ctx) return 0;
  uint64_t n = ctx->st.launches + ctx->aux[0].launches + ctx->aux[1].launches;
  for (const auto& l : ctx->extra) n += l->st.launches + l->aux[0].launches + l->aux[1].launches;
  return n;
}

void* zka_get_stream(zka_ctx* ctx) {
#if !defined(ZKA_HOSTSIM)
  return ctx ? (void*)ctx->st.s : nullptr;
#else
  return nullptr;
#endif
}
int zka_set_profiling(zka_ctx* ctx, int enable) {
  if (!ctx) return ZKA_E_ARG;
  try {
    for (int i = 0; i < 1 + (int)ctx->extra.size(); i++) { sync(ctx->lane(i).st); ctx->lane(i).st.profiling = enable != 0; }
  } catch (...) { return ZKA_E_CUDA; }
  return 0;
}
int zka_profile_reset(zka_ctx* ctx) {
  if (!ctx) return ZKA_E_ARG;
  try {
    for (int i = 0; i < 1 + (int)ctx->extra.size(); i++) { sync(ctx->lane(i).st); ctx->lane(i).st.prof.clear(); }
  } catch (...) { return ZKA_E_CUDA; }
  return 0;
}
int zka_set_option(zka_ctx* ctx, const char* key, long value) {
  if (!ctx || !key || value < 1) return ZKA_E_ARG;
  const std::string k(key);
  return guarded(ctx, [&]() -> int {
    if (k == "lanes") {
      if (value > 8) return ZKA_E_ARG;
      while ((int)ctx->extra.size() + 1 < value) {
        auto l = std::make_unique<Lane>();
        stream_create(l->st);
        stream_create(l->cs_in);
        stream_create(l->cs_out);
        stream_create(l->aux[0]);
        stream_create(l->aux[1]);
        l->st.profiling = ctx->st.profiling;
        ctx->extra.push_back(std::move(l));
      }
      ctx->nlanes = (int)value;
    } else if (k == "chunk") {
      ctx->chunk = (int)value;
    } else if (k == "host_chunk") {
      ctx->host_chunk = (int)value;
    } else if (k == "agg") {
      ctx->agg = (int)value - 1;
    } else if (k == "self_check") {
      if (value > 2) return ZKA_E_ARG;
      ctx->self_check = (int)value - 1;
    } else if (k == "agg_c") {
      if (value < 4 || value > 16) return ZKA_E_ARG;
      ctx->agg_c = (int)value;
    } else {
      return ZKA_E_ARG;
    }
    return 0;
  });
}
long long zka_stat(zka_ctx* ctx, const char* key) {
  if (!ctx || !key) return -1;
  const std::string k(key);
  std::lock_guard<std::mutex> g(ctx->stat_mu);
  if (k == "agg_pass") return (long long)ctx->agg_pass;
  if (k == "agg_fail") return (long long)ctx->agg_fail;
  if (k == "self_check_rows") return (long long)ctx->self_check_rows;
  if (k == "self_check_fail") return (long long)ctx->self_check_fail;
  if (k == "agg_c") return (long long)ctx->agg_c_last;
  if (k == "tom_n_lo") return (long long)ctx->tom.n_lo;
  if (k == "tom_fallback") return ctx->tom_fallback ? 1 : 0;
  return -1;
}
size_t zka_profile_json(zka_ctx* ctx, char* buf, size_t cap) {
  if (!ctx) return 0;
  std::map<std::string, ProfEntry> all;
  try {
    for (int i = 0; i < 1 + (int)ctx->extra.size(); i++) {
      sync(ctx->lane(i).st);
      for (auto& kv : ctx->lane(i).st.prof) {
        ProfEntry& e = all[kv.first];
        e.launches += kv.second.launches; e.ms += kv.second.ms; e.items += kv.second.items;
      }
    }
  } catch (...) { return 0; }
  std::string j = "{";
  bool first = true;
  for (auto& kv : all) {
    char tmp[512];
    snprintf(tmp, sizeof tmp, "%s\"%s\": {\"launches\": %llu, \"ms\": %.6f, \"items\": %llu}", first ? "" : ", ",
             kv.first.c_str(), (unsigned long long)kv.second.launches, kv.second.ms,
             (unsigned long long)kv.second.items);
    j += tmp;
    first = false;
  }
  j += "}";
  if (buf && cap) {
    size_t n = std::min(cap - 1, j.size());
    memcpy(buf, j.data(), n);
    buf[n] = 0;
  }
  return j.size() + 1;
}
#if defined(ZKA_PG_WAR256)
static const char* const PROOF_GROUP = "war256";
#else
static const char* const PROOF_GROUP = "tomEdwards256";
#endif
int zka_proof_group(char* name, size_t cap, int* point_bytes, int* scalar_bytes) {
  const char* n = PROOF_GROUP;
  if (name && cap) {
    strncpy(name, n, cap - 1);
    name[cap - 1] = 0;
  }
  if (point_bytes) *point_bytes = WP;
  if (scalar_bytes) *scalar_bytes = WS;
  return 0;
}
int zka_set_progress(zka_ctx* ctx, volatile uint32_t* flags, uint32_t cap) {
  if (!ctx) return ZKA_E_ARG;
  ctx->progress = flags;
  ctx->progress_cap = flags ? cap : 0;
  return 0;
}
int zka_chunk_schedule(zka_ctx* ctx, uint32_t B, int host_buffers, uint32_t* off, uint32_t cap) {
  if (!ctx || !off || cap == 0) return ZKA_E_ARG;
  const std::vector<uint32_t> v = chunk_schedule(B, (uint32_t)(host_buffers ? std::min(ctx->chunk, ctx->host_chunk) : ctx->chunk), ctx->nlanes,
                                                 host_buffers != 0);
  if (v.size() > cap) return ZKA_E_ARG;
  for (size_t i = 0; i < v.size(); i++) off[i] = v[i];
  return (int)v.size() - 1;
}
int zka_lanes(const zka_ctx* ctx) { return ctx ? ctx->nlanes : 0; }
int zka_config(const zka_ctx* ctx, int* tom_w, int* tom_nwin, int* chunk) {
  if (!ctx) return ZKA_E_ARG;
  if (tom_w) *tom_w = ctx->tom.w;
  if (tom_nwin) *tom_nwin = ctx->tom.nwin;
  if (chunk) *chunk = ctx->chunk;
  return 0;
}

int zka_init(int device, zka_ctx** out) {
  if (!out) return ZKA_E_ARG;
  *out = nullptr;
#if !defined(ZKA_HOSTSIM)
  int ndev = 0;
  cudaError_t e = cudaGetDeviceCount(&ndev);
  if (e != cudaSuccess || ndev == 0 || device >= ndev) {
    cudaGetLastError();
    return ZKA_E_CUDA;
  }
#endif
  std::unique_ptr<zka_ctx> ctx(new zka_ctx());
  const int rc = guarded(ctx.get(), [&] {
#if !defined(ZKA_HOSTSIM)
    ZK_CUDA_CHECK(cudaSetDevice(device));
    ZK_CUDA_CHECK(cudaStreamCreateWithFlags(&ctx->st.s, cudaStreamNonBlocking));
#endif
    ctx->device = device;
    [[maybe_unused]] bool tom_pinned = false;
    if (const char* e = getenv("ZKA_TOM_W")) {
      int w = atoi(e);
      if (w >= 2 && w <= 24) { ctx->tom = fb_uniform(w); tom_pinned = true; }
    }
#if !defined(ZKA_PG_WAR256)
    if (const char* e = tom_pinned ? nullptr : getenv("ZKA_TOM_NWIN")) {
      int n = atoi(e);
      if (n >= 11 && n <= 128) ctx->tom = fb_lookups(n);
    }
#endif
    if (const char* e = getenv("ZKA_TOM_TABLE_MAX")) ctx->tom_table_max = (size_t)strtoull(e, nullptr, 10);
    if (const char* e = getenv("ZKA_CHUNK")) {
      int c = atoi(e);
      if (c >= 1) ctx->chunk = c;
    }
    if (const char* e = getenv("ZKA_NORM_MODEL")) g_norm_model = atoi(e) != 0;
#if !defined(ZKA_HOSTSIM)
    {
      int sms = 0;
      if (cudaDeviceGetAttribute(&sms, cudaDevAttrMultiProcessorCount, device) == cudaSuccess && sms > 0) g_norm_slots = sms * 4;
    }
#endif
    if (const char* e = getenv("ZKA_HOST_CHUNK")) {
      int c = atoi(e);
      if (c >= 1) ctx->host_chunk = c;
    }
    stream_create(ctx->cs_in);
    stream_create(ctx->cs_out);
    stream_create(ctx->aux[0]);
    stream_create(ctx->aux[1]);
    {
      int lanes = 3;
#if defined(ZKA_HOSTSIM)
      lanes = 1;
#endif
      if (const char* e = getenv("ZKA_LANES")) lanes = atoi(e);
      if (lanes < 1) lanes = 1;
      if (lanes > 8) lanes = 8;
      if (zka_set_option(ctx.get(), "lanes", lanes) != 0) throw std::runtime_error("lanes");
    }
    if (const char* e = getenv("ZKA_TAPE_SPLIT")) ctx->tape_split = atoi(e) != 0;
    if (const char* e = getenv("ZKA_AGG")) ctx->agg = atoi(e);
    if (const char* e = getenv("ZKA_AGG_C")) {
      int c = atoi(e);
      if (c >= 4 && c <= 16) ctx->agg_c = c;
    }
    if (const char* e = getenv("ZKA_P256_HW")) {
      int w = atoi(e);
      if (w >= 8 && w <= 24) ctx->p256_hw = w;
    }
    DevBuf gen;
    uint32_t* d_gen = gen.get<uint32_t>(16 + TOM_AFF_WORDS);
    launch(ctx->st, 1, GenAffTask{d_gen, d_gen + 16});
    build_p256_tab(ctx.get(), d_gen, ctx->g8, 8);
    build_p256_tab(ctx.get(), d_gen, ctx->gw, ctx->p256_hw);
#if defined(ZKA_PG_WAR256)
    build_tom_tab(ctx.get(), d_gen + 16, ctx->tg);
#else
    try {
      DevBuf room;
      alloc_tom_tab(ctx.get(), room);
      build_tom_tab(ctx.get(), d_gen + 16, ctx->tg);
    } catch (const std::exception&) {
      if (tom_pinned || ctx->tom.nwin >= 128) throw;
#if !defined(ZKA_HOSTSIM)
      cudaGetLastError();
#endif
      ctx->tg.buf.release();
      ctx->tom = fb_lookups(ctx->tom.nwin + 1);
      ctx->tom_fallback = true;
      build_tom_tab(ctx.get(), d_gen + 16, ctx->tg);
    }
#endif
    DevBuf proj, aff;
    uint32_t* d_proj = proj.get<uint32_t>(TOM_PROJ_WORDS);
    uint32_t* d_aff = aff.get<uint32_t>(TOM_AFF_WORDS);
    uint8_t* d_bytes = ctx->tg_bytes.get<uint8_t>(BSTRIDE);
    launch(ctx->st, 1, GProjTask{d_gen + 16, d_proj});
    launch_tom_norm(ctx->st, d_proj, d_aff, d_bytes, 1, 0);
    sync(ctx->st);
    return 0;
  });
  if (rc) {
    fprintf(stderr, "zka_init: %s\n", ctx->err.c_str());
    return rc;
  }
  *out = ctx.release();
  return 0;
}

void zka_shutdown(zka_ctx* ctx) { delete ctx; }

int zka_params_create(zka_ctx* ctx, const uint8_t h_nist[65], const uint8_t h_proof[67], uint32_t sec_level,
                      zka_params** out) {
  if (!ctx || !h_nist || !h_proof || !out) return ZKA_E_ARG;
  if (sec_level < 1 || sec_level > MAX_REPS) return fail(ctx, ZKA_E_ARG, "sec_level must be in [1,80]");
  return guarded(ctx, [&] {
    std::unique_ptr<zka_params> P(new zka_params());
    P->ctx = ctx;
    P->sec_level = sec_level;
    P->h_w = ctx->p256_hw;
    memcpy(P->h_nist, h_nist, 65);
    memcpy(P->h_proof, h_proof, WP);
    {
      uint8_t name[16] = {};
      memcpy(name, PROOF_GROUP, strlen(PROOF_GROUP));
      Sha256 h;
      h.init();
      sha_tag(h, "ZKAttest/hedge/params/v1");
      h.update(name, 16);
      h.update(h_nist, 65);
      h.update(h_proof, WP);
      h.put4(sec_level);
      alignas(16) uint8_t d[32];
      sha_store(h, d);
      memcpy(P->hedge_digest, d, 32);
    }
    DevBuf bn, bt, an, at, bad, inf;
    uint8_t* d_bn = bn.get<uint8_t>(65);
    uint8_t* d_bt = bt.get<uint8_t>(WP);
    uint32_t* d_an = an.get<uint32_t>(16);
    uint32_t* d_at = at.get<uint32_t>(TOM_AFF_WORDS);
    uint8_t* d_bad = bad.get<uint8_t>(2);
    uint8_t* d_inf = inf.get<uint8_t>(1);
    copy_h2d(ctx->st, d_bn, h_nist, 65);
    copy_h2d(ctx->st, d_bt, h_proof, WP);
    launch(ctx->st, 1, ParsePointsTask{d_bn, nullptr, d_an, nullptr, d_bad, d_inf});
    launch(ctx->st, 1, ParsePointsTask{nullptr, d_bt, nullptr, d_at, d_bad + 1, nullptr});
    uint8_t hb[3];
    copy_d2h(ctx->st, hb, d_bad, 2);
    copy_d2h(ctx->st, hb + 2, d_inf, 1);
    sync(ctx->st);
    if (hb[0] || hb[1] || hb[2]) return fail(ctx, ZKA_E_ARG, "params: h point not on its group");
    build_p256_tab(ctx, d_an, P->h8, P->h_w);
    build_tom_tab(ctx, d_at, P->th);
    *out = P.release();
    return 0;
  });
}

void zka_params_destroy(zka_params* P) { delete P; }

int zka_rings_create(zka_ctx* ctx, uint32_t R, const uint32_t* sizes, const uint8_t* keys, zka_rings** out) {
  if (!ctx || !sizes || !keys || !out) return ZKA_E_ARG;
  *out = nullptr;
  if (R == 0) return fail(ctx, ZKA_E_ARG, "a ring set holds at least one ring");
  if (R > (1u << 23)) return fail(ctx, ZKA_E_ARG, "ring set exceeds 2^24 padded entries");
  std::unique_ptr<zka_rings> set(new zka_rings());
  set->ctx = ctx;
  set->R = R;
  std::vector<uint32_t> key_off(R), base(R);
  uint64_t nkeys = 0, total = 0;
  for (uint32_t r = 0; r < R; r++) {
    const uint32_t N = sizes[r];
    if (N < 2 || N > (1u << 20)) return fail(ctx, ZKA_E_ARG, "ring size must be in [2, 2^20]");
    const int n = ceil_log2(N);
    set->size.push_back(N);
    set->depth.push_back(n);
    key_off[r] = (uint32_t)nkeys;
    base[r] = (uint32_t)total;
    nkeys += N;
    total += 1ull << n;
    if (total > (1ull << 24)) return fail(ctx, ZKA_E_ARG, "ring set exceeds 2^24 padded entries");
  }
  return guarded(ctx, [&] {
    Stream& st = ctx->st;
    DevBuf kbuf, obuf;
    const uint8_t* d_keys = stage_in(st, kbuf, keys, (size_t)nkeys * 32);
    uint32_t* d_off = obuf.get<uint32_t>(R);
    uint32_t* d_base = set->ring_base.get<uint32_t>(R);
    uint32_t* d_size = set->ring_size.get<uint32_t>(R);
    uint32_t* d_depth = set->ring_depth.get<uint32_t>(R);
    const std::vector<uint32_t> depth(set->depth.begin(), set->depth.end());
    const int nmax = *std::max_element(set->depth.begin(), set->depth.end());
    uint32_t* ring_m = set->ring_m.get<uint32_t>((size_t)total * 8);
    copy_h2d(st, d_off, key_off.data(), (size_t)R * 4);
    copy_h2d(st, d_base, base.data(), (size_t)R * 4);
    copy_h2d(st, d_size, set->size.data(), (size_t)R * 4);
    copy_h2d(st, d_depth, depth.data(), (size_t)R * 4);
    launch(st, (long long)total, RingSetPrepTask{d_keys, d_off, d_base, d_size, ring_m, (int)R});
    launch(st, nmax, GkLagrangeSetTask{set->lag.get<uint32_t>(ProveCtx::gk_lag_off(nmax + 1))});
    std::vector<uint32_t> leaf_off(R + 1, 0);
    for (uint32_t r = 0; r < R; r++) leaf_off[r + 1] = leaf_off[r] + hedge_leaves(set->depth[r]);
    DevBuf lbuf, leaves;
    uint32_t* d_leaf_off = lbuf.get<uint32_t>(R + 1);
    copy_h2d(st, d_leaf_off, leaf_off.data(), (size_t)(R + 1) * 4);
    RingDigestTask dt{ring_m, d_base, d_size, d_depth, d_leaf_off, 0u, 0u, R, leaves.get<uint8_t>((size_t)32 * leaf_off[R]),
                      set->ring_digest.get<uint8_t>((size_t)32 * R), false};
    launch(st, leaf_off[R], dt);
    dt.root = true;
    launch(st, R, dt);
    sync(st);
    *out = set.release();
    return 0;
  });
}

void zka_rings_destroy(zka_rings* set) { delete set; }

size_t zka_proof_max_len(uint32_t ring_size, uint32_t sec_level) {
  return (size_t)proof_len((int)sec_level, ceil_log2(ring_size), (int)sec_level);
}
size_t zka_prove_tape_len(uint32_t ring_size, uint32_t sec_level) {
  return (size_t)32 * prove_draws((int)sec_level, ceil_log2(ring_size), (int)sec_level);
}
size_t zka_verify_tape_len(uint32_t ring_size, uint32_t sec_level) {
  return verify_tape_len(ceil_log2(ring_size), (int)sec_level);
}

int zka_tom_commit_batch(zka_ctx* ctx, const zka_params* P, uint32_t count, const uint8_t* v, const uint8_t* r,
                         uint8_t* out) {
  if (!ctx || !P || !v || !r || !out) return ZKA_E_ARG;
  if (count == 0) return 0;
  return guarded(ctx, [&] {
    Stream& st = ctx->st;
    Cursor in(ctx->in[0]), w(ctx->w), ob(ctx->out[0]);
    const uint8_t* dv = stage_in(st, in.next(), v, (size_t)count * 32);
    const uint8_t* dr = stage_in(st, in.next(), r, (size_t)count * 32);
    uint32_t* jv = w.take<uint32_t>((size_t)count * 8);
    uint32_t* jr = w.take<uint32_t>((size_t)count * 8);
    uint32_t* proj = w.take<uint32_t>((size_t)count * TOM_E2_WORDS);
    uint32_t* aff = w.take<uint32_t>((size_t)count * TOM_AFF_WORDS);
    uint8_t* bytes = w.take<uint8_t>((size_t)count * BSTRIDE);
    const Output<uint8_t> o(out, WP);
    uint8_t* packed = o.rows(ob.next(), 0, count);
    launch(st, count, CommitConvTask{dv, dr, jv, jr});
    launch(st, count, TomCommitTask{jv, jr, ctx->tg.tab, P->th.tab, proj, ctx->tom});
    launch_tom_norm(st, proj, aff, bytes, (long long)(count), 1);
    launch(st, count, PackTomTask{bytes, packed});
    o.copy_back(st, 0, packed, count);
    sync(st);
    return 0;
  });
}

int zka_p256_mul_batch(zka_ctx* ctx, uint32_t count, const uint8_t* base, const uint8_t* k, uint8_t* out) {
  if (!ctx || !k || !out) return ZKA_E_ARG;
  if (count == 0) return 0;
  return guarded(ctx, [&] {
    Stream& st = ctx->st;
    Cursor in(ctx->in[0]), w(ctx->w), ob(ctx->out[0]);
    const uint8_t* dk = stage_in(st, in.next(), k, (size_t)count * 32);
    const uint8_t* db = stage_in(st, in.next(), base, (size_t)count * 65);
    uint32_t* proj = w.take<uint32_t>((size_t)count * P256_PROJ_WORDS);
    uint32_t* aff = w.take<uint32_t>((size_t)count * P256_AFF_WORDS);
    uint8_t* bytes = w.take<uint8_t>((size_t)count * BSTRIDE);
    uint8_t* inf = w.take<uint8_t>(count);
    const bool per_base = db != nullptr;
    uint32_t* baff = w.take_if<uint32_t>(per_base, (size_t)count * 16);
    uint8_t* bad = w.take_if<uint8_t>(per_base, count);
    uint8_t* binf = w.take_if<uint8_t>(per_base, count);
    uint32_t* pows = w.take_if<uint32_t>(per_base, (size_t)count * RT_NWIN * P256_PROJ_WORDS);
    uint32_t* rows = w.take_if<uint32_t>(per_base, (size_t)count * RT_ENTRIES * P256_PROJ_WORDS);
    uint32_t* rtab = w.take_if<uint32_t>(per_base, (size_t)count * RT_ENTRIES * P256_AFF_WORDS);
    const Output<uint8_t> o(out, NP);
    uint8_t* packed = o.rows(ob.next(), 0, count);
    if (per_base) {
      launch(st, count, ParsePointsTask{db, nullptr, baff, nullptr, bad, binf});
      launch(st, count, P256PowsTask{baff, binf, pows, (int)count, RT_NWIN, RT_W});
      launch(st, (long long)count * RT_NWIN, P256RowsSignedTask{pows, rows});
      const long long np = (long long)count * RT_ENTRIES;
      launch_p256_norm(st, rows, rtab, nullptr, nullptr, (long long)(np));
    }
    launch(st, count, P256MulTask{dk, ctx->g8.tab, rtab, binf, proj});
    launch_p256_norm(st, proj, aff, bytes, inf, (long long)(count));
    launch(st, count, PackP256Task{bytes, packed});
    o.copy_back(st, 0, packed, count);
    sync(st);
    return 0;
  });
}


int zka_field_op_batch(zka_ctx* ctx, int field, int op, uint32_t count, const uint8_t* a, const uint8_t* b,
                       uint8_t* out) {
  if (!ctx || !a || !out || field < 0 || field > 2 || op < 0 || op > 4 || (op < 3 && !b)) return ZKA_E_ARG;
  if (count == 0) return 0;
  return guarded(ctx, [&] {
    Stream& st = ctx->st;
    Cursor in(ctx->in[0]), ob(ctx->out[0]);
    const int nb = field == 2 ? WCB : 32;
    const uint8_t* da = stage_in(st, in.next(), a, (size_t)count * nb);
    const uint8_t* db = stage_in(st, in.next(), b, (size_t)count * nb);
    const Output<uint8_t> o(out, nb);
    uint8_t* dout = o.rows(ob.next(), 0, count);
    if (field == 0) launch(st, count, FieldOpTask<P256p, 32>{da, db, dout, op});
    else if (field == 1) launch(st, count, FieldOpTask<P256n, 32>{da, db, dout, op});
    else launch(st, count, FieldOpTask<PGp, WCB>{da, db, dout, op});
    o.copy_back(st, 0, dout, count);
    sync(st);
    return 0;
  });
}

int zka_hash80_batch(zka_ctx* ctx, uint32_t count, const uint8_t* msgs, size_t msg_stride, const uint32_t* len,
                     uint8_t* out) {
  if (!ctx || !msgs || !len || !out) return ZKA_E_ARG;
  if (count == 0) return 0;
  return guarded(ctx, [&] {
    Stream& st = ctx->st;
    Cursor in(ctx->in[0]), ob(ctx->out[0]);
    const uint8_t* dm = stage_in(st, in.next(), msgs, (size_t)count * msg_stride);
    const uint32_t* dl = stage_in(st, in.next(), len, (size_t)count);
    const Output<uint8_t> o(out, 10);
    uint8_t* dout = o.rows(ob.next(), 0, count);
    launch(st, count, Hash80Task{dm, msg_stride, dl, dout});
    o.copy_back(st, 0, dout, count);
    sync(st);
    return 0;
  });
}

int zka_params_generate(zka_ctx* ctx, const uint8_t rnd[64], uint8_t h_nist[65], uint8_t h_proof[67]) {
  if (!ctx || !rnd || !h_nist || !h_proof) return ZKA_E_ARG;
  return guarded(ctx, [&] {
    int rc = zka_p256_mul_batch(ctx, 1, nullptr, rnd, h_nist);
    if (rc) return rc;
    Stream& st = ctx->st;
    Cursor in(ctx->in[0]), w(ctx->w);
    uint32_t* jv = w.take<uint32_t>(8);
    uint32_t* jr = w.take<uint32_t>(8);
    uint32_t* proj = w.take<uint32_t>(TOM_E2_WORDS);
    uint32_t* aff = w.take<uint32_t>(TOM_AFF_WORDS);
    uint8_t* bytes = w.take<uint8_t>(BSTRIDE);
    uint8_t* d_rnd = in.take<uint8_t>(32);
    copy_h2d(st, d_rnd, rnd + 32, 32);
    launch(st, 1, GenConvTask{d_rnd, jv, jr});
    launch(st, 1, TomCommitTask{jv, jr, ctx->tg.tab, ctx->tg.tab, proj, ctx->tom});
    launch_tom_norm(st, proj, aff, bytes, (long long)(1), 1);
    copy_d2h(st, h_proof, bytes, WP);
    sync(st);
    return 0;
  });
}

int zka_key_to_int(zka_ctx* ctx, uint32_t count, const uint8_t* pk, uint8_t* x_out, int32_t* status) {
  if (!ctx || !pk || !x_out) return ZKA_E_ARG;
  if (count == 0) return 0;
  return guarded(ctx, [&] {
    Stream& st = ctx->st;
    Cursor in(ctx->in[0]), w(ctx->w), ob(ctx->out[0]);
    const uint8_t* dp = stage_in(st, in.next(), pk, (size_t)count * 65);
    uint32_t* aff = w.take<uint32_t>((size_t)count * 16);
    uint8_t* bad = w.take<uint8_t>(count);
    uint8_t* inf = w.take<uint8_t>(count);
    const Output<uint8_t> xo(x_out, 32);
    const Output<int32_t> so(status, 1);
    uint8_t* dx = xo.rows(ob.next(), 0, count);
    int32_t* ds = so.rows(ob.next(), 0, count);
    launch(st, count, ParsePointsTask{dp, nullptr, aff, nullptr, bad, inf});
    launch(st, count, KeyToIntTask{aff, bad, inf, dx, ds});
    xo.copy_back(st, 0, dx, count);
    if (status) so.copy_back(st, 0, ds, count);
    sync(st);
    return 0;
  });
}

static int prove_impl(zka_ctx* ctx, const zka_params* P, uint32_t B, const ProveRows& rows, const RingSrc& ring, int mode) {
  const int S = (int)P->sec_level, n = ring.n;
  const bool hedge = rows.hedge, seeded = rows.seeds != nullptr || hedge;
  const bool check = ctx->self_check && mode == 0;
  const int seed_draws = prove_draws(S, n, S);
  const uint32_t* ring_m = ring.prepare(ctx, true, hedge);
  const uint8_t* ring_digest = hedge ? ring.digests(ctx) : nullptr;
  const Output<uint8_t> po(rows.proofs, rows.proof_stride);
  const Output<uint32_t> lo(rows.proof_len, 1);
  const Output<int32_t> so(rows.status, 1);
  const int lanes = ctx->nlanes;
  const size_t dev_tape_stride = (rows.tape_stride + 15) & ~(size_t)15;
  const uint8_t* rnd_in = seeded ? rows.seeds : rows.tape;
  const bool all_dev = po.dev && (!rnd_in || is_device_ptr(rnd_in));
  const std::vector<uint32_t> off = chunk_schedule(B, (uint32_t)(all_dev ? ctx->chunk : std::min(ctx->chunk, ctx->host_chunk)), lanes, !all_dev);
  const uint32_t nchunks = (uint32_t)off.size() - 1;
  const int used = (int)std::min<uint32_t>((uint32_t)lanes, nchunks);
  const bool trace = getenv("ZKA_TRACE") != nullptr;
  const auto t_call = std::chrono::steady_clock::now();
  auto ms_now = [&] { return std::chrono::duration<double, std::milli>(std::chrono::steady_clock::now() - t_call).count(); };
  std::atomic<uint32_t> next_chunk((uint32_t)used);
  auto run_lane = [&](int li) {
    Lane& ln = ctx->lane(li);
    Stream& st = ln.st;
    ProveRows cin[2];
    uint32_t* check_counts = check ? ln.chk_count.get<uint32_t>(2) : nullptr;
    if (check) dev_memset(st, check_counts, 0, 8);
    auto issue_inputs = [&](uint32_t k, int slot) {
      const ProveRows r = rows.at(off[k]), e = rows.at(off[k + 1]);
      const size_t Bc = off[k + 1] - off[k];
      Stream& ci = ln.cs_in;
      Cursor in(ln.in[slot]);
      DevBuf& tape_buf = in.next();
      auto stage = [&](auto* p, auto* end) { return stage_in(ci, in.next(), p, (size_t)(end - p)); };
      ev_wait(ci, ln.ev_done[slot]);
      ProveRows& d = cin[slot];
      d.msg_hash = stage(r.msg_hash, e.msg_hash);
      d.sig = stage(r.sig, e.sig);
      d.pk = stage(r.pk, e.pk);
      d.which = stage(r.which, e.which);
      d.ring_of = stage(r.ring_of, e.ring_of);
      d.base = stage(r.base, e.base);
      d.s_in = stage(r.s_in, e.s_in);
      d.q_in = stage(r.q_in, e.q_in);
      d.seeds = stage(r.seeds, e.seeds);
      ev_record(ln.ev_small[slot], ci);
      if (seeded) {
        d.tape = tape_buf.get<uint8_t>(Bc * (size_t)32 * seed_draws);
      } else if (is_device_ptr(rows.tape)) {
        d.tape = r.tape;
      } else if (!ctx->tape_split && dev_tape_stride == rows.tape_stride) {
        d.tape = stage_in(ci, tape_buf, r.tape, (size_t)(e.tape - r.tape));
      } else {
// ... 339 lines not shown
int zka_prove_membership_batch(zka_ctx* ctx, const zka_params* P, uint32_t B, const uint8_t* com_r, const uint32_t* index,
                               const uint8_t* ring, uint32_t N, const uint8_t* tape, size_t tape_stride, uint8_t* proofs,
                               size_t proof_stride, uint32_t* proof_len, int32_t* status) {
  if (!ctx || !P || !com_r || !index || !ring || !tape || !proofs || !proof_len || !status) return ZKA_E_ARG;
  if (B == 0) return 0;
  if (N < 2 || N > (1u << 20)) return fail(ctx, ZKA_E_ARG, "ring size must be in [2, 2^20]");
  const int n = ceil_log2(N);
  if (proof_stride < (size_t)gk_len(n)) return fail(ctx, ZKA_E_ARG, "proof_stride < GK block length");
  if (tape_stride < (size_t)32 * 5 * n) return fail(ctx, ZKA_E_ARG, "tape_stride < 32 * 5n");
  return guarded(ctx, [&] {
    Stream& st = ctx->st;
    const uint32_t* ring_m = prep_ring(ctx, st, ring, N, n, true);
    const Output<uint8_t> po(proofs, proof_stride);
    const Output<uint32_t> lo(proof_len, 1);
    const Output<int32_t> so(status, 1);
    const size_t it_len = 96 + tape_stride, it_stride = (it_len + 15) & ~(size_t)15;
    const uint32_t chunk = 8192;
    for (uint32_t b0 = 0; b0 < B; b0 += chunk) {
      const int Bc = (int)std::min<uint32_t>(chunk, B - b0);
      Cursor in(ctx->in[0]), w(ctx->w), ob(ctx->out[0]);
      const uint8_t* d_cr = stage_in(st, in.next(), com_r + (size_t)b0 * 32, (size_t)Bc * 32);
      const uint32_t* d_idx = stage_in(st, in.next(), index + b0, (size_t)Bc);
      const uint8_t* d_tape = stage_in(st, in.next(), tape + (size_t)b0 * tape_stride, (size_t)Bc * tape_stride);
      ProveCtx c = prove_ctx(ctx, P, Bc, 0, (int)N, n);
      c.which = d_idx;
      c.ring_m = ring_m;
      uint8_t* itape = w.take<uint8_t>((size_t)Bc * it_stride);
      c.tape = itape; c.tape_stride = it_stride; c.tape_draws = (uint32_t)(it_len / 32);
      c.which_s = w.take<uint32_t>(Bc);
      c.zcount = w.take<uint32_t>(Bc);
      c.gk_off = w.take<uint32_t>(Bc);
      c.gk_dv = w.take<uint32_t>((size_t)Bc * n * 8);
      c.gk_x = w.take<uint32_t>((size_t)Bc * 3);
      const size_t ng = (size_t)Bc * 4 * n;
      c.s2_jv = w.take<uint32_t>(ng * 8);
      c.s2_jr = w.take<uint32_t>(ng * 8);
      c.s2_proj = w.take<uint32_t>(ng * TOM_E2_WORDS);
      c.s2_bytes = w.take<uint8_t>(ng * BSTRIDE);
      c.gk_part = w.take_if<uint32_t>(gk_blocks(n) > 1, (size_t)Bc * n * gk_blocks(n) * 8);
      c.proof_stride = proof_stride;
      c.proofs = po.rows(ob.next(), b0, Bc);
      c.proof_len = lo.rows(ob.next(), b0, Bc);
      c.status = so.rows(ob.next(), b0, Bc);
      uint32_t* gext = w.take<uint32_t>(prove_gext_words(c));
      launch(st, Bc, GkAloneSetupTask{c, d_cr, d_tape, tape_stride, itape});
      prove_items_gk(st, c, gext, false, true);
      launch(st, Bc, GkEmitTask{c});
      launch(st, (long long)Bc * FIN_PARTS, FinalizeTask{c});
      po.copy_back_2d(st, b0, c.proofs, Bc, (size_t)gk_len(n));
      lo.copy_back(st, b0, c.proof_len, Bc);
      so.copy_back(st, b0, c.status, Bc);
      sync(st);
    }
    return 0;
  });
}

static int prove_sub(zka_ctx* ctx, const zka_params* P, int kind, uint32_t B, const uint8_t* scalars, const uint8_t* tape,
                     size_t tape_stride, uint8_t* commitments, uint8_t* proofs, int32_t* status) {
  if (!ctx || !P || !scalars || !tape || !commitments || !proofs || !status) return ZKA_E_ARG;
  if (B == 0) return 0;
  const int ns = kind == 0 ? 3 : 6, nd = kind == 0 ? 3 : 7, J = kind == 0 ? SUBP_EQ_JOBS : SUBP_MULT_JOBS;
  const int nc = kind == 0 ? 2 : 3, plen = kind == 0 ? EQ_LEN : MULT_LEN;
  if (tape_stride < (size_t)32 * nd) return fail(ctx, ZKA_E_ARG, "tape_stride too small for this sub-proof");
  return guarded(ctx, [&] {
    Stream& st = ctx->st;
    const Output<uint8_t> co(commitments, (size_t)nc * WP), po(proofs, plen);
    const Output<int32_t> so(status, 1);
    const uint32_t chunk = 16384;
    for (uint32_t b0 = 0; b0 < B; b0 += chunk) {
      const int Bc = (int)std::min<uint32_t>(chunk, B - b0);
      Cursor in(ctx->in[0]), w(ctx->w), ob(ctx->out[0]);
      const uint8_t* d_sc = stage_in(st, in.next(), scalars + (size_t)b0 * ns * 32, (size_t)Bc * ns * 32);
      const uint8_t* d_tape = stage_in(st, in.next(), tape + (size_t)b0 * tape_stride, (size_t)Bc * tape_stride);
      const size_t nj = (size_t)Bc * J;
      uint32_t* jv = w.take<uint32_t>(nj * 8);
      uint32_t* jr = w.take<uint32_t>(nj * 8);
      uint32_t* proj = w.take<uint32_t>(nj * TOM_E2_WORDS);
      uint8_t* bytes = w.take<uint8_t>(nj * BSTRIDE);
      uint8_t* d_com = co.rows(ob.next(), b0, Bc);
      uint8_t* d_prf = po.rows(ob.next(), b0, Bc);
      int32_t* d_st = so.rows(ob.next(), b0, Bc);
      launch(st, Bc, SubProveJobsTask{kind, d_sc, d_tape, tape_stride, jv, jr, d_st});
      launch(st, (long long)nj, TomCommitTask{jv, jr, ctx->tg.tab, P->th.tab, proj, ctx->tom});
      launch_tom_norm(st, proj, nullptr, bytes, (long long)nj, 1);
      launch(st, Bc, SubProveEmitTask{kind, d_sc, d_tape, tape_stride, jr, bytes, d_com, d_prf, d_st});
      co.copy_back(st, b0, d_com, Bc);
      po.copy_back(st, b0, d_prf, Bc);
      so.copy_back(st, b0, d_st, Bc);
      sync(st);
    }
    return 0;
  });
}
int zka_prove_equality_batch(zka_ctx* ctx, const zka_params* P, uint32_t B, const uint8_t* scalars, const uint8_t* tape,
                             size_t tape_stride, uint8_t* commitments, uint8_t* proofs, int32_t* status) {
  return prove_sub(ctx, P, 0, B, scalars, tape, tape_stride, commitments, proofs, status);
}
int zka_prove_mult_batch(zka_ctx* ctx, const zka_params* P, uint32_t B, const uint8_t* scalars, const uint8_t* tape,
                         size_t tape_stride, uint8_t* commitments, uint8_t* proofs, int32_t* status) {
  return prove_sub(ctx, P, 1, B, scalars, tape, tape_stride, commitments, proofs, status);
}

int zka_prove_pointadd_batch(zka_ctx* ctx, const zka_params* P, uint32_t B, const uint8_t* points, const uint8_t* blinders,
                             const uint8_t* tape, size_t tape_stride, uint8_t* commitments, uint8_t* proofs, int32_t* status) {
  if (!ctx || !P || !points || !blinders || !tape || !commitments || !proofs || !status) return ZKA_E_ARG;
  if (B == 0) return 0;
  if (tape_stride < (size_t)32 * 38) return fail(ctx, ZKA_E_ARG, "tape_stride < 32 * 38");
  return guarded(ctx, [&] {
    Stream& st = ctx->st;
    const size_t it_stride = (size_t)32 * (9 + 38);
    const size_t row_stride = REP0_LEN;
    const Output<uint8_t> co(commitments, 6 * WP), po(proofs, PA_LEN);
    const Output<int32_t> so(status, 1);
    const uint32_t chunk = 8192;
    for (uint32_t b0 = 0; b0 < B; b0 += chunk) {
      const int Bc = (int)std::min<uint32_t>(chunk, B - b0);
      Cursor in(ctx->in[0]), w(ctx->w), ob(ctx->out[0]);
      const uint8_t* d_pts = stage_in(st, in.next(), points + (size_t)b0 * 195, (size_t)Bc * 195);
      const uint8_t* d_bl = stage_in(st, in.next(), blinders + (size_t)b0 * 192, (size_t)Bc * 192);
      const uint8_t* d_tape = stage_in(st, in.next(), tape + (size_t)b0 * tape_stride, (size_t)Bc * tape_stride);
      ProveCtx c = prove_ctx(ctx, P, Bc, 1, 2, 0);
      c.M = Bc; c.mode = 1; c.head_len = 0;
      uint8_t* itape = w.take<uint8_t>((size_t)Bc * it_stride);
      c.tape = itape; c.tape_stride = it_stride; c.tape_draws = (uint32_t)(it_stride / 32);
      const size_t n1 = (size_t)Bc * 4, n2 = (size_t)Bc * (JOBS_PER_ITEM + DERS_PER_ITEM);
      c.s1 = w.take<uint32_t>((size_t)Bc * 8);
      c.pk_aff = w.take<uint32_t>((size_t)Bc * 16);
      c.pa_T_aff = w.take<uint32_t>((size_t)Bc * 2 * 16);
      c.pa_T_inf = w.take<uint8_t>((size_t)Bc * 2);
      c.pa_A_inf = w.take<uint8_t>((size_t)Bc * 2);
      c.pb_T1_aff = w.take<uint32_t>((size_t)Bc * 16);
      c.pb_T1_inf = w.take<uint8_t>(Bc);
      c.chal = w.take<uint32_t>((size_t)Bc * 3);
      c.zcount = w.take<uint32_t>(Bc);
      c.item_base = w.take<uint32_t>(Bc);
      c.item_b = w.take<uint32_t>(Bc);
      c.item_i = w.take<uint32_t>(Bc);
      c.item_k = w.take<uint32_t>(Bc);
      c.rep_off = w.take<uint32_t>(Bc);
      c.s1_jv = w.take<uint32_t>(n1 * 8);
      c.s1_jr = w.take<uint32_t>(n1 * 8);
      c.s1_proj = w.take<uint32_t>(n1 * TOM_E2_WORDS);
      c.s1_aff = w.take<uint32_t>(n1 * TOM_AFF_WORDS);
      c.s1_bytes = w.take<uint8_t>(n1 * BSTRIDE);
      c.s2_jv = w.take<uint32_t>(n2 * 8);
      c.s2_jr = w.take<uint32_t>(n2 * 8);
      c.s2_proj = w.take<uint32_t>(n2 * TOM_E2_WORDS);
      c.s2_aff = w.take<uint32_t>(n2 * TOM_AFF_WORDS);
      c.s2_bytes = w.take<uint8_t>(n2 * BSTRIDE);
      c.secrets = w.take<uint32_t>((size_t)Bc * SECRETS_PER_ITEM * 8);
      c.item_inv = w.take<uint32_t>((size_t)Bc * 8);
      c.item_chal = w.take<uint32_t>((size_t)Bc * HASHES_PER_ITEM * 3);
      uint32_t* gext = w.take<uint32_t>(prove_gext_words(c));
      c.proof_stride = row_stride;
      c.proofs = w.take<uint8_t>((size_t)Bc * row_stride);
      c.proof_len = w.take<uint32_t>(Bc);
      uint8_t* d_com = co.rows(ob.next(), b0, Bc);
      uint8_t* d_prf = po.rows(ob.next(), b0, Bc);
      c.status = so.rows(ob.next(), b0, Bc);
      launch(st, Bc, PaddSetupTask{c, d_pts, d_bl, d_tape, tape_stride, itape});
      prove_store1(st, c);
      prove_items_gk(st, c, gext, true, false);
      launch(st, Bc, PaddExtractTask{c, d_com, d_prf});
      co.copy_back(st, b0, d_com, Bc);
      po.copy_back(st, b0, d_prf, Bc);
      so.copy_back(st, b0, c.status, Bc);
// ... 166 lines not shown
  return verify_batch(ctx, P, B, r, RingSrc::pass(rings, 0), samples, 0);
}

int zka_verify_exp_batch(zka_ctx* ctx, const zka_params* P, uint32_t B, const uint8_t* base, const uint8_t* com,
                         const uint8_t* px, const uint8_t* py, const uint8_t* q, const uint8_t* proofs, size_t proof_stride,
                         const uint32_t* proof_len, const uint8_t* tape, size_t tape_stride, uint32_t samples, uint8_t* ok,
                         int32_t* status) {
  if (!ctx || !P || !base || !com || !px || !py || !proofs || !proof_len || !tape || !ok || !status || proof_stride == 0) return ZKA_E_ARG;
  if (B == 0) return 0;
  return guarded(ctx, [&] {
    Stream& st = ctx->st;
    DevBuf bufs[10];
    Cursor in(bufs);
    const uint8_t* d_base = stage_in(st, in.next(), base, (size_t)B * NP);
    const uint8_t* d_com = stage_in(st, in.next(), com, (size_t)B * NP);
    const uint8_t* d_px = stage_in(st, in.next(), px, (size_t)B * WP);
    const uint8_t* d_py = stage_in(st, in.next(), py, (size_t)B * WP);
    const uint8_t* d_q = stage_in(st, in.next(), q, (size_t)B * NP);
    const uint8_t* d_body = stage_in(st, in.next(), proofs, (size_t)B * proof_stride);
    const uint32_t* d_len = stage_in(st, in.next(), proof_len, (size_t)B);
    const uint8_t* d_tape = stage_in(st, in.next(), tape, (size_t)B * tape_stride);
    const size_t row_stride = (HEAD_LEN + proof_stride + 15) & ~(size_t)15;
    uint8_t* d_rows = in.take<uint8_t>((size_t)B * row_stride);
    uint32_t* d_rlen = in.take<uint32_t>(B);
    const int pieces = (int)((row_stride + 63) / 64);
    launch(st, (long long)B * pieces, VAssembleTask{d_base, d_com, d_px, d_py, d_body, proof_stride, d_len, d_rows, row_stride, d_rlen, pieces});
    sync(st);
    VerifyRows r(d_rows, row_stride, d_rlen, ok, status);
    r.tape = d_tape; r.tape_stride = tape_stride; r.q_ext = d_q;
    return verify_batch(ctx, P, B, r, RingSrc::none(1), samples, 1);
  });
}

int zka_verify_membership_batch(zka_ctx* ctx, const zka_params* P, uint32_t B, const uint8_t* com, const uint8_t* ring, uint32_t N,
                                const uint8_t* proofs, size_t proof_stride, const uint32_t* proof_len, const uint8_t* tape,
                                size_t tape_stride, uint8_t* ok, int32_t* status) {
  if (!ctx || !P || !com || !ring || !proofs || !proof_len || !tape || !ok || !status || proof_stride == 0) return ZKA_E_ARG;
  if (B == 0) return 0;
  if (N < 2 || N > (1u << 20)) return fail(ctx, ZKA_E_ARG, "ring size must be in [2, 2^20]");
  const int n = ceil_log2(N);
  if (tape_stride < (size_t)32 * (2 * n + 1)) return fail(ctx, ZKA_E_ARG, "tape_stride < 32 * (2n + 1)");
  return guarded(ctx, [&] {
    Stream& st = ctx->st;
    DevBuf bufs[4];
    const uint32_t* ring_m = prep_ring(ctx, st, ring, N, n, false);
    const Output<uint8_t> oo(ok, 1);
    const Output<int32_t> so(status, 1);
    const size_t row_stride = (HEAD_LEN + proof_stride + 15) & ~(size_t)15;
    const int pieces = (int)((row_stride + 63) / 64);
    const int ngk = 4 * n + 1;
    const uint32_t chunk = 4096;
    for (uint32_t b0 = 0; b0 < B; b0 += chunk) {
      const int Bc = (int)std::min<uint32_t>(chunk, B - b0);
      Cursor in(bufs), w(ctx->w), ob(ctx->out[0]);
      const uint8_t* d_com = stage_in(st, in.next(), com + (size_t)b0 * WP, (size_t)Bc * WP);
      const uint8_t* d_body = stage_in(st, in.next(), proofs + (size_t)b0 * proof_stride, (size_t)Bc * proof_stride);
      const uint32_t* d_len = stage_in(st, in.next(), proof_len + b0, (size_t)Bc);
      VerifyCtx c = verify_ctx(ctx, P, Bc, (int)P->sec_level, (int)N, n, 1, 2);
      c.tape = stage_in(st, in.next(), tape + (size_t)b0 * tape_stride, (size_t)Bc * tape_stride);
      c.tape_stride = tape_stride;
      c.ring_m = ring_m;
      uint8_t* d_rows = w.take<uint8_t>((size_t)Bc * row_stride);
      uint32_t* d_rlen = w.take<uint32_t>(Bc);
      c.proofs = d_rows; c.proof_stride = row_stride; c.proof_len = d_rlen;
      c.gk_off = w.take<uint32_t>(Bc);
      c.gk_ok_len = w.take<uint8_t>(Bc);
      c.gk_scalar = w.take<uint32_t>((size_t)Bc * ngk * 8);
      c.gk_pre = w.take<uint32_t>((size_t)Bc * ngk * TOM_PRE_WORDS);
      uint32_t* gk_offs = w.take<uint32_t>((size_t)Bc * ngk);
      c.fx_jv = w.take<uint32_t>((size_t)Bc * 2 * 8);
      c.fx_jr = w.take<uint32_t>((size_t)Bc * 2 * 8);
      c.fx_proj = w.take<uint32_t>((size_t)Bc * 2 * TOM_PROJ_WORDS);
      c.win_g = w.take<uint32_t>((size_t)Bc * MSM_NWIN * 36);
      c.id_flags = w.take<uint8_t>((size_t)Bc * 3);
      c.gk_part = w.take_if<uint32_t>(gk_blocks(n) > 1, (size_t)Bc * gk_blocks(n) * 8);
      c.ok = oo.rows(ob.next(), b0, Bc);
      c.status = so.rows(ob.next(), b0, Bc);
      launch(st, (long long)Bc * pieces, VAssembleTask{nullptr, nullptr, d_com, nullptr, d_body, proof_stride, d_len, d_rows, row_stride, d_rlen, pieces});
      launch(st, Bc, VGkOnlyLayoutTask{c});
      dev_memset(st, c.fx_jv, 0, (size_t)Bc * 2 * 8 * 4);
      dev_memset(st, c.fx_jr, 0, (size_t)Bc * 2 * 8 * 4);
      verify_gk(st, c, gk_offs);
      launch(st, (long long)Bc * ngk, VParseEntriesTask{c.proofs, row_stride, gk_offs, c.gk_pre, ngk});
      launch(st, (long long)Bc * 2, TomCommitTask{c.fx_jv, c.fx_jr, c.tg_tab, c.th_tab, c.fx_proj, c.tom, 1});
      launch(st, (long long)Bc * MSM_NWIN, MsmTomWindowTask{c.gk_scalar, c.gk_pre, nullptr, ngk, 0, 0, ngk, V_SEG, 1, c.win_g});
      launch(st, Bc, MsmTomCombineTask{c.win_g, c.fx_proj, c.id_flags, 2, 0, 0});
      launch(st, Bc, VGkOnlyFinalTask{c});
      oo.copy_back(st, b0, c.ok, Bc);
      so.copy_back(st, b0, c.status, Bc);
      sync(st);
    }
    return 0;
  });
}

static int verify_sub(zka_ctx* ctx, const zka_params* P, int kind, uint32_t B, const uint8_t* points, const uint8_t* proofs,
                      const uint8_t* tape, size_t tape_stride, uint8_t* ok, int32_t* status) {
  if (!ctx || !P || !points || !proofs || !tape || !ok || !status) return ZKA_E_ARG;
  if (B == 0) return 0;
  if (tape_stride < (size_t)32 * sub_draws(kind)) return fail(ctx, ZKA_E_ARG, "tape_stride too small for this sub-proof");
  return guarded(ctx, [&] {
    Stream& st = ctx->st;
    const int la = sub_points(kind) * WP, lc = sub_proof_len(kind), ne = sub_entries(kind);
    const size_t stride = (size_t)(la + lc + 15) & ~(size_t)15;
    const Output<uint8_t> oo(ok, 1);
    const Output<int32_t> so(status, 1);
    const uint32_t chunk = 8192;
    for (uint32_t b0 = 0; b0 < B; b0 += chunk) {
      const int Bc = (int)std::min<uint32_t>(chunk, B - b0);
      Cursor in(ctx->in[0]), w(ctx->w), ob(ctx->out[0]);
      const uint8_t* d_pts = stage_in(st, in.next(), points + (size_t)b0 * la, (size_t)Bc * la);
      const uint8_t* d_prf = stage_in(st, in.next(), proofs + (size_t)b0 * lc, (size_t)Bc * lc);
      const uint8_t* d_tape = stage_in(st, in.next(), tape + (size_t)b0 * tape_stride, (size_t)Bc * tape_stride);
      uint8_t* rows = w.take<uint8_t>((size_t)Bc * stride);
      uint32_t* ent_scalar = w.take<uint32_t>((size_t)Bc * SUB_ENT_MAX * 8);
      uint32_t* ent_off = w.take<uint32_t>((size_t)Bc * SUB_ENT_MAX);
      uint32_t* ent_pre = w.take<uint32_t>((size_t)Bc * SUB_ENT_MAX * TOM_PRE_WORDS);
      uint32_t* fx_jv = w.take<uint32_t>((size_t)Bc * 2 * 8);
      uint32_t* fx_jr = w.take<uint32_t>((size_t)Bc * 2 * 8);
      uint32_t* fx_proj = w.take<uint32_t>((size_t)Bc * 2 * TOM_PROJ_WORDS);
      uint32_t* win = w.take<uint32_t>((size_t)Bc * MSM_NWIN * 36);
      uint8_t* flags = w.take<uint8_t>((size_t)Bc * 3);
      uint8_t* d_ok = oo.rows(ob.next(), b0, Bc);
      int32_t* d_st = so.rows(ob.next(), b0, Bc);
      launch(st, (long long)Bc * (la + lc), VConcatTask{d_pts, d_prf, la, lc, rows, stride});
      launch(st, Bc, VSubProofTask{kind, rows, stride, d_tape, tape_stride, (const uint8_t*)ctx->tg_bytes.p, ent_scalar, ent_off,
                                   fx_jv, fx_jr, d_st, d_ok});
      launch(st, (long long)Bc * SUB_ENT_MAX, VParseEntriesTask{rows, stride, ent_off, ent_pre, SUB_ENT_MAX});
      launch(st, (long long)Bc * 2, TomCommitTask{fx_jv, fx_jr, ctx->tg.tab, P->th.tab, fx_proj, ctx->tom, 1});
      launch(st, (long long)Bc * MSM_NWIN, MsmTomWindowTask{ent_scalar, ent_pre, nullptr, SUB_ENT_MAX, 0, 0, ne, V_SEG, 1, win});
      launch(st, Bc, MsmTomCombineTask{win, fx_proj, flags, 2, 1, 1});
      launch(st, Bc, VSubFinalTask{d_st, flags, d_ok});
      oo.copy_back(st, b0, d_ok, Bc);
      so.copy_back(st, b0, d_st, Bc);
      sync(st);
    }
    return 0;
  });
}
int zka_verify_equality_batch(zka_ctx* ctx, const zka_params* P, uint32_t B, const uint8_t* points, const uint8_t* proofs,
                              const uint8_t* tape, size_t tape_stride, uint8_t* ok, int32_t* status) {
  return verify_sub(ctx, P, SUB_EQ, B, points, proofs, tape, tape_stride, ok, status);
}
int zka_verify_mult_batch(zka_ctx* ctx, const zka_params* P, uint32_t B, const uint8_t* points, const uint8_t* proofs,
                          const uint8_t* tape, size_t tape_stride, uint8_t* ok, int32_t* status) {
  return verify_sub(ctx, P, SUB_MULT, B, points, proofs, tape, tape_stride, ok, status);
}
int zka_verify_pointadd_batch(zka_ctx* ctx, const zka_params* P, uint32_t B, const uint8_t* points, const uint8_t* proofs,
                              const uint8_t* tape, size_t tape_stride, uint8_t* ok, int32_t* status) {
  return verify_sub(ctx, P, SUB_PADD, B, points, proofs, tape, tape_stride, ok, status);
}

namespace {
int pack_common(zka_ctx* ctx, uint32_t B, uint8_t* rows, size_t stride, const uint32_t* len, uint8_t* packed, size_t cap,
                uint64_t* offsets, void* stream, int dir) {
  if (!ctx || !rows || !len || !packed || !offsets || stride == 0) return ZKA_E_ARG;
  if (B == 0) return 0;
#if !defined(ZKA_HOSTSIM)
  if (!is_device_ptr(rows) || !is_device_ptr(len) || !is_device_ptr(packed) || !is_device_ptr(offsets))
    return fail(ctx, ZKA_E_ARG, "zka_proofs_pack/unpack take device pointers");
#endif
  return guarded(ctx, [&] {
    Stream tmp;
    Stream* st = &ctx->st;
#if !defined(ZKA_HOSTSIM)
    if (stream) { tmp.s = (cudaStream_t)stream; st = &tmp; }
#endif
    const int pieces = (int)((stride + 15) / 16);
    launch(*st, 1, PackScanTask{len, offsets, (int)B});
    const bool al = (stride % 16 == 0) && (((size_t)rows | (size_t)packed) % 16 == 0);
    if (al) launch(*st, (long long)B * pieces, PackCopy16Task{rows, stride, len, offsets, packed, cap, pieces, dir});
    else launch(*st, (long long)B * pieces, PackCopyTask{rows, stride, len, offsets, packed, cap, pieces, dir});
    if (st == &tmp) ctx->st.launches += tmp.launches; else sync(*st);
    return 0;
  });
}
}

int zka_proofs_pack(zka_ctx* ctx, uint32_t B, const uint8_t* proofs, size_t proof_stride, const uint32_t* proof_len,
                    uint8_t* packed, size_t cap, uint64_t* offsets, void* stream) {
  return pack_common(ctx, B, const_cast<uint8_t*>(proofs), proof_stride, proof_len, packed, cap, offsets, stream, 0);
}
int zka_proofs_unpack(zka_ctx* ctx, uint32_t B, const uint8_t* packed, size_t cap, const uint32_t* proof_len, uint8_t* proofs,
                      size_t proof_stride, uint64_t* offsets, void* stream) {
  return pack_common(ctx, B, proofs, proof_stride, proof_len, const_cast<uint8_t*>(packed), cap, offsets, stream, 1);
}

}
```

Baseline: 122,000.

## Give the H-base fixed-base table its own larger window shape

Splits the single Tom fixed-base table shape into separate G and H shapes. By default the per-params H table is built with 10 windows (wider windows, fewer lookups and point additions per commitment) when enough free device memory remains after a per-lane reserve. Otherwise it falls back to the shared shape. Commit kernels interleave G and H digits across the differing window counts. The cost is a much larger H table that uses device memory and setup time, and possibly more cache pressure on random table loads.

```diff
diff --git a/__graft_entry__.py b/__graft_entry__.py
--- a/__graft_entry__.py
+++ b/__graft_entry__.py
@@ -23,6 +23,9 @@
 PROBE_SHAPE_SRC = os.path.join(ROOT, 'tests', 'probe', 'zk_probe_shape.cu')
 PROBE_SHAPE = os.path.join(ROOT, 'tests', 'probe', 'libzkprobe_shape.so')
 PROBE_SHAPE_HOST = os.path.join(ROOT, 'tests', 'probe', 'libzkprobe_shape_host.so')
+PROBE_SHAPE_H_SRC = os.path.join(ROOT, 'tests', 'probe', 'zk_probe_shape_h.cu')
+PROBE_SHAPE_H = os.path.join(ROOT, 'tests', 'probe', 'libzkprobe_shape_h.so')
+PROBE_SHAPE_H_HOST = os.path.join(ROOT, 'tests', 'probe', 'libzkprobe_shape_h_host.so')
 ORACLE_CPU = os.path.join(ROOT, 'oracle', '_ref', 'libzkattest_cpu.so')
 ARCH = ['-gencode', 'arch=compute_90a,code=sm_90a']
 NVCC_FLAGS = ARCH + ['-O3', '-std=c++17', '-lineinfo',
@@ -99,14 +102,16 @@
     return _build_if_stale(out, cmd, 'probe_seed' + (' host (tests only)' if host else ' (sm_90a, tests only)'), [PROBE_SEED_SRC])
 
 
-def build_probe_shape(host=False):
-    out = PROBE_SHAPE_HOST if host else PROBE_SHAPE
+def build_probe_shape(host=False, h=False):
+    out = (PROBE_SHAPE_H_HOST if host else PROBE_SHAPE_H) if h else (PROBE_SHAPE_HOST if host else PROBE_SHAPE)
+    src = PROBE_SHAPE_H_SRC if h else PROBE_SHAPE_SRC
     if host:
         cmd = ['g++', '-std=c++17', '-O2', '-DZKA_HOSTSIM', '-x', 'c++', '-fPIC', '-shared']
     else:
         cmd = [os.environ.get('NVCC', '/usr/local/cuda/bin/nvcc')] + NVCC_FLAGS
-    cmd += ['-I' + os.path.join(ROOT, 'include'), '-I' + CSRC, '-o', out, PROBE_SHAPE_SRC]
-    return _build_if_stale(out, cmd, 'probe_shape' + (' host (tests only)' if host else ' (sm_90a, tests only)'), [PROBE_SHAPE_SRC])
+    cmd += ['-I' + os.path.join(ROOT, 'include'), '-I' + CSRC, '-o', out, src]
+    tag = ('probe_shape_h' if h else 'probe_shape') + (' host (tests only)' if host else ' (sm_90a, tests only)')
+    return _build_if_stale(out, cmd, tag, [PROBE_SHAPE_SRC, PROBE_SHAPE_H_SRC] if h else [PROBE_SHAPE_SRC])
 
 
 def build_oracle_cpu():
@@ -139,7 +144,8 @@
     jobs = [build_lib, build_lib_war, build_hostsim, lambda: build_hostsim(war=True), build_oracle_cpu, build_tools,
             build_probe, lambda: build_probe(host=True), lambda: build_probe(jac=True),
             lambda: build_probe(host=True, jac=True), build_probe_seed, lambda: build_probe_seed(host=True),
-            build_probe_shape, lambda: build_probe_shape(host=True)]
+            build_probe_shape, lambda: build_probe_shape(host=True), lambda: build_probe_shape(h=True),
+            lambda: build_probe_shape(host=True, h=True)]
     with ThreadPoolExecutor(max_workers=min(len(jobs), max(1, (os.cpu_count() or 2)))) as ex:
         for f in [ex.submit(j) for j in jobs]:
             f.result()
diff --git a/zkp_ecdsa_b200/capi.py b/zkp_ecdsa_b200/capi.py
--- a/zkp_ecdsa_b200/capi.py
+++ b/zkp_ecdsa_b200/capi.py
@@ -212,6 +212,9 @@
         cfg = {'tom_w': w.value, 'tom_nwin': nw.value, 'chunk': ch.value, 'lanes': lanes}
         if hasattr(self.lib, 'zka_stat') and self.stat('tom_n_lo') >= 0:
             cfg.update(tom_n_lo=self.stat('tom_n_lo'), tom_fallback=bool(self.stat('tom_fallback')))
+        if hasattr(self.lib, 'zka_stat') and self.stat('tom_h_nwin') >= 0:
+            cfg.update(tom_h_w=self.stat('tom_h_w'), tom_h_nwin=self.stat('tom_h_nwin'), tom_h_n_lo=self.stat('tom_h_n_lo'),
+                       tom_h_fallback=bool(self.stat('tom_h_fallback')))
         return cfg
 
     def set_option(self, key: str, value: int):
diff --git a/zkp_ecdsa_b200/csrc/zk_launch.cuh b/zkp_ecdsa_b200/csrc/zk_launch.cuh
--- a/zkp_ecdsa_b200/csrc/zk_launch.cuh
+++ b/zkp_ecdsa_b200/csrc/zk_launch.cuh
@@ -13,6 +13,8 @@
 
 #if !defined(ZKA_HOSTSIM)
 #include <cuda_runtime.h>
+#else
+#include <unistd.h>
 #endif
 
 namespace zk {
@@ -138,6 +140,11 @@
   if (ev.e) cudaEventDestroy(ev.e);
   ev.e = nullptr;
 }
+inline size_t dev_free_bytes() {
+  size_t free = 0, total = 0;
+  ZK_CUDA_CHECK(cudaMemGetInfo(&free, &total));
+  return free;
+}
 inline bool is_device_ptr(const void* p) {
   cudaPointerAttributes a;
   cudaError_t e = cudaPointerGetAttributes(&a, p);
@@ -182,6 +189,7 @@
 inline void ev_wait(Stream&, Event&) {}
 inline void ev_destroy(Event&) {}
 inline bool is_device_ptr(const void*) { return false; }
+inline size_t dev_free_bytes() { return (size_t)sysconf(_SC_AVPHYS_PAGES) * (size_t)sysconf(_SC_PAGE_SIZE); }
 
 #endif
 
diff --git a/zkp_ecdsa_b200/csrc/zk_ops.cuh b/zkp_ecdsa_b200/csrc/zk_ops.cuh
--- a/zkp_ecdsa_b200/csrc/zk_ops.cuh
+++ b/zkp_ecdsa_b200/csrc/zk_ops.cuh
@@ -584,26 +584,32 @@
   const uint32_t* gtab;
   const uint32_t* htab;
   uint32_t* proj;
-  FbShape sh;
+  FbShape gsh, hsh;
   int xyz = 0;
   ZK_HD void operator()(int t) const {
     uint32_t v[8], r[8];
     ld<8>(v, jv + (size_t)t * 8);
     ld<8>(r, jr + (size_t)t * 8);
     uint32_t cv = 0, cr = 0;
-    bool nv, nr;
+    bool neg;
     TomPre q;
-    uint32_t dv = signed_digit(v, 0, sh, cv, nv);
-    tom2_ld_entry(q, gtab, sh, 0, dv, nv);
+    uint32_t d = signed_digit(v, 0, gsh, cv, neg);
+    tom2_ld_entry(q, gtab, gsh, 0, d, neg);
     TomPt acc;
     tom2_from_pre(acc, q);
-    for (int j = 0;; j++) {
-      const uint32_t dr = signed_digit(r, j, sh, cr, nr);
-      tom2_ld_entry(q, htab, sh, j, dr, nr);
-      if (j == sh.nwin - 1) break;
-      tom2_madd<true>(acc, acc, q);
-      dv = signed_digit(v, j + 1, sh, cv, nv);
-      tom2_ld_entry(q, gtab, sh, j + 1, dv, nv);
+    const int m = gsh.nwin < hsh.nwin ? gsh.nwin : hsh.nwin, last = gsh.nwin + hsh.nwin - 1;
+    const bool h_longer = hsh.nwin > gsh.nwin;
+    for (int i = 1;; i++) {
+      const bool h = i < 2 * m ? (i & 1) != 0 : h_longer;
+      const int j = i < 2 * m ? i >> 1 : i - m;
+      if (h) {
+        d = signed_digit(r, j, hsh, cr, neg);
+        tom2_ld_entry(q, htab, hsh, j, d, neg);
+      } else {
+        d = signed_digit(v, j, gsh, cv, neg);
+        tom2_ld_entry(q, gtab, gsh, j, d, neg);
+      }
+      if (i == last) break;
       tom2_madd<true>(acc, acc, q);
     }
     if (xyz) {
@@ -652,7 +658,7 @@
   const uint32_t* htab;
   const uint32_t* ext;
   uint32_t* proj;
-  FbShape sh;
+  FbShape gsh, hsh;
   GpartLayout lay;
   ZK_HD void operator()(int t) const {
     const int row = t / lay.jobs(), g = lay.gpart_of_job(row, t % lay.jobs());
@@ -661,7 +667,7 @@
     TomPt acc;
     TomPre q;
     if (g < 0 || scalar_le_one(v)) {
-      tom2_ld_entry(q, gtab, sh, 0, v[0], false);
+      tom2_ld_entry(q, gtab, gsh, 0, v[0], false);
       tom2_from_pre<TompCommit>(acc, q);
     } else {
       const uint32_t* s = ext + ((size_t)row * lay.gparts() + g) * TOM_EXT_WORDS;
@@ -671,13 +677,13 @@
     uint32_t carry = 0;
     bool neg;
 #pragma unroll 1
-    for (int j = 0; j < sh.nwin - 1; j++) {
-      const uint32_t d = signed_digit(r, j, sh, carry, neg);
-      tom2_ld_entry(q, htab, sh, j, d, neg);
+    for (int j = 0; j < hsh.nwin - 1; j++) {
+      const uint32_t d = signed_digit(r, j, hsh, carry, neg);
+      tom2_ld_entry(q, htab, hsh, j, d, neg);
       tom2_madd<true, TompCommit>(acc, acc, q);
     }
-    const uint32_t d = signed_digit(r, sh.nwin - 1, sh, carry, neg);
-    tom2_ld_entry(q, htab, sh, sh.nwin - 1, d, neg);
+    const uint32_t d = signed_digit(r, hsh.nwin - 1, hsh, carry, neg);
+    tom2_ld_entry(q, htab, hsh, hsh.nwin - 1, d, neg);
     TomEfgh e;
     tom2_madd_end<TompCommit>(e, acc, q);
     tom_st_efgh(proj + (size_t)t * TOM_E2_WORDS, e);
diff --git a/zkp_ecdsa_b200/csrc/zk_ops_war.cuh b/zkp_ecdsa_b200/csrc/zk_ops_war.cuh
--- a/zkp_ecdsa_b200/csrc/zk_ops_war.cuh
+++ b/zkp_ecdsa_b200/csrc/zk_ops_war.cuh
@@ -76,7 +76,7 @@
   const uint32_t* gtab;
   const uint32_t* htab;
   uint32_t* proj;
-  FbShape sh;
+  FbShape gsh, hsh;
   int xyz = 0;
   ZK_HD void operator()(int t) const {
     uint32_t v[8], r[8];
@@ -84,8 +84,8 @@
     ld<8>(r, jr + (size_t)t * 8);
     WarJac aj;
     war_set_identity_jac(aj);
-    war_accum_fixed_jac(aj, gtab, v, sh.w);
-    war_accum_fixed_jac(aj, htab, r, sh.w);
+    war_accum_fixed_jac(aj, gtab, v, gsh.w);
+    war_accum_fixed_jac(aj, htab, r, hsh.w);
     WarPt acc;
     war_jac_to_hom(acc, aj);
     war_st_proj(proj + (size_t)t * TOM_PROJ_WORDS, acc);
@@ -120,7 +120,7 @@
   const uint32_t* htab;
   const uint32_t* ext;
   uint32_t* proj;
-  FbShape sh;
+  FbShape gsh, hsh;
   GpartLayout lay;
   ZK_HD void operator()(int t) const {
     const int row = t / lay.jobs(), g = lay.gpart_of_job(row, t % lay.jobs());
@@ -128,9 +128,9 @@
     ld<8>(v, jv + (size_t)t * 8);
     ld<8>(r, jr + (size_t)t * 8);
     WarPt acc;
-    if (g < 0 || scalar_le_one(v)) war_gpart(acc, gtab, v, sh.w);
+    if (g < 0 || scalar_le_one(v)) war_gpart(acc, gtab, v, gsh.w);
     else war_ld_proj(acc, ext + ((size_t)row * lay.gparts() + g) * TOM_EXT_WORDS);
-    war_accum_fixed(acc, htab, r, sh.w);
+    war_accum_fixed(acc, htab, r, hsh.w);
     war_st_proj(proj + (size_t)t * TOM_PROJ_WORDS, acc);
   }
 };
diff --git a/zkp_ecdsa_b200/csrc/zk_prove.cuh b/zkp_ecdsa_b200/csrc/zk_prove.cuh
--- a/zkp_ecdsa_b200/csrc/zk_prove.cuh
+++ b/zkp_ecdsa_b200/csrc/zk_prove.cuh
@@ -9,7 +9,7 @@
   int N;
   int n;
   int M;
-  FbShape tom;
+  FbShape tom_g, tom_h;
   int mode;
   int head_len;
   const uint8_t* base;
diff --git a/zkp_ecdsa_b200/csrc/zk_verify.cuh b/zkp_ecdsa_b200/csrc/zk_verify.cuh
--- a/zkp_ecdsa_b200/csrc/zk_verify.cuh
+++ b/zkp_ecdsa_b200/csrc/zk_verify.cuh
@@ -33,7 +33,7 @@
   int K;
   int mode;
   const uint8_t* q_ext;
-  FbShape tom;
+  FbShape tom_g, tom_h;
   const uint8_t* msg_hash;
   const uint8_t* proofs;
   size_t proof_stride;
diff --git a/zkp_ecdsa_b200/csrc/zkattest.cu b/zkp_ecdsa_b200/csrc/zkattest.cu
--- a/zkp_ecdsa_b200/csrc/zkattest.cu
+++ b/zkp_ecdsa_b200/csrc/zkattest.cu
@@ -300,6 +300,14 @@
 #endif
   size_t tom_table_max = 0;
   bool tom_fallback = false;
+#if defined(ZKA_PG_WAR256)
+  int tom_h_nwin = 0;
+#else
+  int tom_h_nwin = 10;
+#endif
+  long long tom_h_reserve = -1;
+  FbShape tom_h_last{};
+  bool tom_h_fallback = false;
   int chunk = 4096;
   int host_chunk = 2048;
   volatile uint32_t* progress = nullptr;
@@ -328,6 +336,7 @@
   FixedTable h8;
   int h_w = 20;
   FixedTable th;
+  FbShape tom_h{};
   uint8_t h_nist[65];
   uint8_t h_proof[WP];
   uint8_t hedge_digest[32];
@@ -450,21 +459,22 @@
   launch_p256_norm(st, d_rows, out.tab, nullptr, nullptr, (long long)(count));
   sync(st);
 }
-uint32_t* alloc_tom_tab(zka_ctx* ctx, DevBuf& buf) {
-  const size_t words = ctx->tom.total() * TOM_PRE_WORDS;
+constexpr size_t TOM_H_RESERVE_PER_ROW = (size_t)2 << 20;
+uint32_t* alloc_tom_tab(zka_ctx* ctx, const FbShape& sh, DevBuf& buf) {
+  const size_t words = sh.total() * TOM_PRE_WORDS;
   if (ctx->tom_table_max && words * sizeof(uint32_t) > ctx->tom_table_max)
     throw std::runtime_error("proof-group fixed-base table of " + std::to_string(words * sizeof(uint32_t)) + " bytes exceeds ZKA_TOM_TABLE_MAX");
   return buf.get_exact<uint32_t>(words);
 }
 #if defined(ZKA_PG_WAR256)
-void build_tom_tab(zka_ctx* ctx, const uint32_t* base_aff_dev, FixedTable& out) {
+void build_tom_tab(zka_ctx* ctx, const FbShape& sh, const uint32_t* base_aff_dev, FixedTable& out) {
   Stream& st = ctx->st;
-  const int w = ctx->tom.w, nwin = ctx->tom.nwin;
+  const int w = sh.w, nwin = sh.nwin;
   const size_t E = (size_t)fb_entries(w), count = (size_t)nwin * E;
   DevBuf pows, rows;
   uint32_t* d_pows = pows.get<uint32_t>((size_t)nwin * P256_PROJ_WORDS);
   uint32_t* d_rows = rows.get<uint32_t>(count * P256_PROJ_WORDS);
-  out.tab = alloc_tom_tab(ctx, out.buf);
+  out.tab = alloc_tom_tab(ctx, sh, out.buf);
   launch(st, 1, WarPowsTask{base_aff_dev, nullptr, d_pows, 1, nwin, w});
   if (w > 9) {
     DevBuf hi;
@@ -483,10 +493,9 @@
   sync(st);
 }
 #else
-void build_tom_tab(zka_ctx* ctx, const uint32_t* base_aff_dev, FixedTable& out) {
+void build_tom_tab(zka_ctx* ctx, const FbShape& sh, const uint32_t* base_aff_dev, FixedTable& out) {
   Stream& st = ctx->st;
-  const FbShape sh = ctx->tom;
-  out.tab = alloc_tom_tab(ctx, out.buf);
+  out.tab = alloc_tom_tab(ctx, sh, out.buf);
   DevBuf pows, rows, hi;
   uint32_t* d_pows = pows.get<uint32_t>((size_t)sh.nwin * 36);
   uint32_t* d_rows = rows.get<uint32_t>(sh.entries(sh.nwin - 1) * TOM_PROJ_WORDS);
@@ -712,7 +721,8 @@
   ProveCtx c;
   memset(&c, 0, sizeof(c));
   c.B = B; c.S = S; c.N = N; c.n = n;
-  c.tom = ctx->tom;
+  c.tom_g = ctx->tom;
+  c.tom_h = P->tom_h;
   c.g_tab8 = ctx->g8.tab; c.h_tab8 = P->h8.tab; c.h_w = P->h_w;
   c.g_tabw = ctx->gw.tab; c.g_w = ctx->p256_hw;
   c.tg_tab = ctx->tg.tab; c.th_tab = P->th.tab;
@@ -724,7 +734,8 @@
   VerifyCtx c;
   memset(&c, 0, sizeof(c));
   c.B = B; c.S = S; c.N = N; c.n = n; c.K = K; c.mode = mode;
-  c.tom = ctx->tom;
+  c.tom_g = ctx->tom;
+  c.tom_h = P->tom_h;
   c.g_tab8 = ctx->g8.tab; c.h_tab8 = P->h8.tab; c.h_w = P->h_w;
   c.tg_tab = ctx->tg.tab; c.th_tab = P->th.tab;
   c.tg_bytes = (const uint8_t*)ctx->tg_bytes.p;
@@ -734,7 +745,7 @@
 void prove_store1(Stream& st, const ProveCtx& c) {
   const long long n1 = (long long)c.B * (2 + 2 * c.S);
   launch(st, n1, JobsATask{c});
-  launch(st, n1, TomCommitTask{c.s1_jv, c.s1_jr, c.tg_tab, c.th_tab, c.s1_proj, c.tom});
+  launch(st, n1, TomCommitTask{c.s1_jv, c.s1_jr, c.tg_tab, c.th_tab, c.s1_proj, c.tom_g, c.tom_h});
   launch_tom_norm(st, c.s1_proj, c.s1_aff, c.s1_bytes, n1, 1);
 }
 size_t prove_gext_words(const ProveCtx& c) { return ((size_t)c.M * GJOBS_PER_ITEM + (size_t)c.B * 2 * c.n) * TOM_EXT_WORDS; }
@@ -756,13 +767,13 @@
     launch(st, Bn, GkCdJobsTask{c});
   }
   if (items) {
-    launch(st, M * GJOBS_PER_ITEM, TomCommitGTask{c.s2_jv, c.tg_tab, gext, c.tom, item_lay});
-    launch(st, nj, TomCommitHTask{c.s2_jv, c.s2_jr, c.tg_tab, c.th_tab, gext, c.s2_proj, c.tom, item_lay});
+    launch(st, M * GJOBS_PER_ITEM, TomCommitGTask{c.s2_jv, c.tg_tab, gext, c.tom_g, item_lay});
+    launch(st, nj, TomCommitHTask{c.s2_jv, c.s2_jr, c.tg_tab, c.th_tab, gext, c.s2_proj, c.tom_g, c.tom_h, item_lay});
   }
   if (gk) {
-    launch(st, 2 * Bn, TomCommitGTask{c.s2_jv + g0 * 8, c.tg_tab, gk_ext, c.tom, gk_lay});
+    launch(st, 2 * Bn, TomCommitGTask{c.s2_jv + g0 * 8, c.tg_tab, gk_ext, c.tom_g, gk_lay});
     launch(st, ng, TomCommitHTask{c.s2_jv + g0 * 8, c.s2_jr + g0 * 8, c.tg_tab, c.th_tab, gk_ext, c.s2_proj + g0 * TOM_E2_WORDS,
-                                  c.tom, gk_lay});
+                                  c.tom_g, c.tom_h, gk_lay});
   }
   if (items) {
     launch_tom_norm(st, c.s2_proj, c.s2_aff, c.s2_bytes, nj, 1, JOBS_PER_ITEM, 2);
@@ -871,7 +882,7 @@
   launch(st, (long long)ns, VSampleP256Task{c});
   launch_p256_norm(st, c.sp_T, c.sp_T_aff, nullptr, c.sp_T_inf, (long long)(ns));
   launch(st, (long long)ns, VSampleJobsTask{c});
-  launch(st, (long long)ns * 2, TomCommitTask{c.ta_jv, c.ta_jr, c.tg_tab, c.th_tab, c.ta_proj, c.tom});
+  launch(st, (long long)ns * 2, TomCommitTask{c.ta_jv, c.ta_jr, c.tg_tab, c.th_tab, c.ta_proj, c.tom_g, c.tom_h});
   launch_tom_norm(st, c.ta_proj, c.ta_aff, nullptr, (long long)(ns * 2), 1);
   launch(st, (long long)ns, VDerivedTask{c});
   launch_tom_norm(st, c.td_proj, nullptr, c.td_bytes, (long long)(ns * DERS_PER_ITEM), 0);
@@ -885,7 +896,7 @@
   launch(st, Bc, VReduceTask{c});
   launch(st, (long long)Bc * ET, VParseEntriesTask{c.proofs, c.proof_stride, c.ent_off, c.ent_pre, ET});
   if (mode == 0) launch(st, (long long)Bc * ngk, VParseEntriesTask{c.proofs, c.proof_stride, gk_offs, c.gk_pre, ngk});
-  launch(st, (long long)Bc * 2, TomCommitTask{c.fx_jv, c.fx_jr, c.tg_tab, c.th_tab, c.fx_proj, c.tom, 1});
+  launch(st, (long long)Bc * 2, TomCommitTask{c.fx_jv, c.fx_jr, c.tg_tab, c.th_tab, c.fx_proj, c.tom_g, c.tom_h, 1});
   uint32_t* ctl = nullptr;
   if (agg) {
     Cursor A(ln.agg);
@@ -925,7 +936,7 @@
     agg_msm(sb, Cursor(ln.agg_nist), nsrc, np, ctl, &nA, &nB);
     launch(st, fgroups, AggFixPartTask{ctl, c.fx_jv, c.fx_jr, agg_wt, fpart, Bc});
     launch(st, 1, AggFixSumTask{ctl, fpart, fjv, fjr, fgroups});
-    launch(st, 1, TomCommitTask{fjv, fjr, c.tg_tab, c.th_tab, fproj, c.tom, 1});
+    launch(st, 1, TomCommitTask{fjv, fjr, c.tg_tab, c.th_tab, fproj, c.tom_g, c.tom_h, 1});
     launch(sb, Bc, AggNistFixWeightTask{ctl, c.nfix_k, agg_wt, c.rtab, c.h_tab8, c.h_w, nfix_w});
     launch(sb, ngroups, AggNistFixPartTask{ctl, nfix_w, npart, Bc});
     int nleft = ngroups;
@@ -1071,6 +1082,10 @@
   if (k == "agg_c") return (long long)ctx->agg_c_last;
   if (k == "tom_n_lo") return (long long)ctx->tom.n_lo;
   if (k == "tom_fallback") return ctx->tom_fallback ? 1 : 0;
+  if (k == "tom_h_w") return (long long)ctx->tom_h_last.w;
+  if (k == "tom_h_nwin") return (long long)ctx->tom_h_last.nwin;
+  if (k == "tom_h_n_lo") return (long long)ctx->tom_h_last.n_lo;
+  if (k == "tom_h_fallback") return ctx->tom_h_fallback ? 1 : 0;
   return -1;
 }
 size_t zka_profile_json(zka_ctx* ctx, char* buf, size_t cap) {
@@ -1169,6 +1184,14 @@
       int n = atoi(e);
       if (n >= 11 && n <= 128) ctx->tom = fb_lookups(n);
     }
+#endif
+#if !defined(ZKA_PG_WAR256)
+    if (getenv("ZKA_TOM_W") || getenv("ZKA_TOM_NWIN")) ctx->tom_h_nwin = 0;
+    if (const char* e = getenv("ZKA_TOM_H_NWIN")) {
+      int n = atoi(e);
+      if (n >= 10 && n <= 128) ctx->tom_h_nwin = n;
+    }
+    if (const char* e = getenv("ZKA_TOM_H_RESERVE")) ctx->tom_h_reserve = (long long)strtoull(e, nullptr, 10);
 #endif
     if (const char* e = getenv("ZKA_TOM_TABLE_MAX")) ctx->tom_table_max = (size_t)strtoull(e, nullptr, 10);
     if (const char* e = getenv("ZKA_CHUNK")) {
@@ -1216,12 +1239,12 @@
     build_p256_tab(ctx.get(), d_gen, ctx->g8, 8);
     build_p256_tab(ctx.get(), d_gen, ctx->gw, ctx->p256_hw);
 #if defined(ZKA_PG_WAR256)
-    build_tom_tab(ctx.get(), d_gen + 16, ctx->tg);
+    build_tom_tab(ctx.get(), ctx->tom, d_gen + 16, ctx->tg);
 #else
     try {
       DevBuf room;
-      alloc_tom_tab(ctx.get(), room);
-      build_tom_tab(ctx.get(), d_gen + 16, ctx->tg);
+      alloc_tom_tab(ctx.get(), ctx->tom, room);
+      build_tom_tab(ctx.get(), ctx->tom, d_gen + 16, ctx->tg);
     } catch (const std::exception&) {
       if (tom_pinned || ctx->tom.nwin >= 128) throw;
 #if !defined(ZKA_HOSTSIM)
@@ -1230,9 +1253,10 @@
       ctx->tg.buf.release();
       ctx->tom = fb_lookups(ctx->tom.nwin + 1);
       ctx->tom_fallback = true;
-      build_tom_tab(ctx.get(), d_gen + 16, ctx->tg);
+      build_tom_tab(ctx.get(), ctx->tom, d_gen + 16, ctx->tg);
     }
 #endif
+    ctx->tom_h_last = ctx->tom;
     DevBuf proj, aff;
     uint32_t* d_proj = proj.get<uint32_t>(TOM_PROJ_WORDS);
     uint32_t* d_aff = aff.get<uint32_t>(TOM_AFF_WORDS);
@@ -1294,7 +1318,34 @@
     sync(ctx->st);
     if (hb[0] || hb[1] || hb[2]) return fail(ctx, ZKA_E_ARG, "params: h point not on its group");
     build_p256_tab(ctx, d_an, P->h8, P->h_w);
-    build_tom_tab(ctx, d_at, P->th);
+    bool own = false;
+    if (ctx->tom_h_nwin) {
+      const FbShape sh = fb_lookups(ctx->tom_h_nwin);
+      const size_t reserve = ctx->tom_h_reserve >= 0 ? (size_t)ctx->tom_h_reserve
+                                                     : (size_t)ctx->nlanes * (size_t)ctx->chunk * TOM_H_RESERVE_PER_ROW;
+      if (dev_free_bytes() >= sh.total() * TOM_PRE_WORDS * sizeof(uint32_t) + reserve) {
+        try {
+          build_tom_tab(ctx, sh, d_at, P->th);
+          P->tom_h = sh;
+          own = true;
+        } catch (const std::exception&) {
+#if !defined(ZKA_HOSTSIM)
+          cudaGetLastError();
+#endif
+          P->th.buf.release();
+          P->th.tab = nullptr;
+        }
+      }
+    }
+    if (!own) {
+      build_tom_tab(ctx, ctx->tom, d_at, P->th);
+      P->tom_h = ctx->tom;
+    }
+    {
+      std::lock_guard<std::mutex> g(ctx->stat_mu);
+      ctx->tom_h_last = P->tom_h;
+      ctx->tom_h_fallback = ctx->tom_h_nwin && !own;
+    }
     *out = P.release();
     return 0;
   });
@@ -1386,7 +1437,7 @@
     const Output<uint8_t> o(out, WP);
     uint8_t* packed = o.rows(ob.next(), 0, count);
     launch(st, count, CommitConvTask{dv, dr, jv, jr});
-    launch(st, count, TomCommitTask{jv, jr, ctx->tg.tab, P->th.tab, proj, ctx->tom});
+    launch(st, count, TomCommitTask{jv, jr, ctx->tg.tab, P->th.tab, proj, ctx->tom, P->tom_h});
     launch_tom_norm(st, proj, aff, bytes, (long long)(count), 1);
     launch(st, count, PackTomTask{bytes, packed});
     o.copy_back(st, 0, packed, count);
@@ -1487,7 +1538,7 @@
     uint8_t* d_rnd = in.take<uint8_t>(32);
     copy_h2d(st, d_rnd, rnd + 32, 32);
     launch(st, 1, GenConvTask{d_rnd, jv, jr});
-    launch(st, 1, TomCommitTask{jv, jr, ctx->tg.tab, ctx->tg.tab, proj, ctx->tom});
+    launch(st, 1, TomCommitTask{jv, jr, ctx->tg.tab, ctx->tg.tab, proj, ctx->tom, ctx->tom});
     launch_tom_norm(st, proj, aff, bytes, (long long)(1), 1);
     copy_d2h(st, h_proof, bytes, WP);
     sync(st);
@@ -1993,7 +2044,7 @@
       uint8_t* d_prf = po.rows(ob.next(), b0, Bc);
       int32_t* d_st = so.rows(ob.next(), b0, Bc);
       launch(st, Bc, SubProveJobsTask{kind, d_sc, d_tape, tape_stride, jv, jr, d_st});
-      launch(st, (long long)nj, TomCommitTask{jv, jr, ctx->tg.tab, P->th.tab, proj, ctx->tom});
+      launch(st, (long long)nj, TomCommitTask{jv, jr, ctx->tg.tab, P->th.tab, proj, ctx->tom, P->tom_h});
       launch_tom_norm(st, proj, nullptr, bytes, (long long)nj, 1);
       launch(st, Bc, SubProveEmitTask{kind, d_sc, d_tape, tape_stride, jr, bytes, d_com, d_prf, d_st});
       co.copy_back(st, b0, d_com, Bc);
@@ -2326,7 +2377,7 @@
       dev_memset(st, c.fx_jr, 0, (size_t)Bc * 2 * 8 * 4);
       verify_gk(st, c, gk_offs);
       launch(st, (long long)Bc * ngk, VParseEntriesTask{c.proofs, row_stride, gk_offs, c.gk_pre, ngk});
-      launch(st, (long long)Bc * 2, TomCommitTask{c.fx_jv, c.fx_jr, c.tg_tab, c.th_tab, c.fx_proj, c.tom, 1});
+      launch(st, (long long)Bc * 2, TomCommitTask{c.fx_jv, c.fx_jr, c.tg_tab, c.th_tab, c.fx_proj, c.tom_g, c.tom_h, 1});
       launch(st, (long long)Bc * MSM_NWIN, MsmTomWindowTask{c.gk_scalar, c.gk_pre, nullptr, ngk, 0, 0, ngk, V_SEG, 1, c.win_g});
       launch(st, Bc, MsmTomCombineTask{c.win_g, c.fx_proj, c.id_flags, 2, 0, 0});
       launch(st, Bc, VGkOnlyFinalTask{c});
@@ -2371,7 +2422,7 @@
       launch(st, Bc, VSubProofTask{kind, rows, stride, d_tape, tape_stride, (const uint8_t*)ctx->tg_bytes.p, ent_scalar, ent_off,
                                    fx_jv, fx_jr, d_st, d_ok});
       launch(st, (long long)Bc * SUB_ENT_MAX, VParseEntriesTask{rows, stride, ent_off, ent_pre, SUB_ENT_MAX});
-      launch(st, (long long)Bc * 2, TomCommitTask{fx_jv, fx_jr, ctx->tg.tab, P->th.tab, fx_proj, ctx->tom, 1});
+      launch(st, (long long)Bc * 2, TomCommitTask{fx_jv, fx_jr, ctx->tg.tab, P->th.tab, fx_proj, ctx->tom, P->tom_h, 1});
       launch(st, (long long)Bc * MSM_NWIN, MsmTomWindowTask{ent_scalar, ent_pre, nullptr, SUB_ENT_MAX, 0, 0, ne, V_SEG, 1, win});
       launch(st, Bc, MsmTomCombineTask{win, fx_proj, flags, 2, 1, 1});
       launch(st, Bc, VSubFinalTask{d_st, flags, d_ok});
```

Result: faster. 125,300, median of 6 (+2.7%).
